# lppllppl920/SAGE-SLAM

Measured on AMD Instinct MI355X. Metric: M residuals/sec (+ LM iters/sec), 64-keyframe feature-metric BA @128x160, higher is better.
Workload: dtype f32; 1 GPU; 64-keyframe window, 128x160x16 feature pyramids (L=4), 32-dim depth code, dense sampling N=16128, 186 links = 372 photometric + 372 geometric directed edges; parallelism=single GPU, collective=none, accepted_steps=988

## Files before the change

include/sage_ba.h:

```cpp
#ifndef SAGE_BA_H_
#define SAGE_BA_H_

#include <stddef.h>
#include <stdint.h>

#ifdef __cplusplus
extern "C" {
#endif

#define SAGE_MAX_LEVELS 8
#define SAGE_POSE_FLOATS 12

#define SAGE_OK 0
#define SAGE_E_INVALID (-1)
#define SAGE_E_UNSUPPORTED (-2)
#define SAGE_E_NOT_PSD (-3)
#define SAGE_E_STATE (-4)
#define SAGE_E_NO_OVERLAP (-5)

typedef struct SageCamera
{
  float fx, fy, cx, cy, w, h;
} SageCamera;

// ... 621 lines not shown
                                        const float *matched_2d, const SageCamera *cam, float eps, float loss_param,
                                        float weight, int N);

enum { SAGE_LOSS_FAIR = 0, SAGE_LOSS_L2 = 1, SAGE_LOSS_HUBER = 2, SAGE_LOSS_UNBIASED = 3 };
int sage_match_geometry_jac_error_calculate(SageWorkspace *ws, float *AtA_dev, float *Atb_dev, float *error_host,
                                            const float *R10, const float *t10, const float *R0, const float *t0,
                                            const float *R1, const float *t1, const float *bias0, const float *bias1,
                                            const float *basis0, const float *basis1, const float *code0,
                                            const float *code1, const float *homo0, const float *matched_homo1,
                                            const int32_t *loc1d_0, const int32_t *matched_loc1d_1, float scale0,
                                            float scale1, float loss_param, float weight, int loss, int N, int CS);
int sage_match_geometry_error_calculate(SageWorkspace *ws, float *error_host, const float *R10, const float *t10,
                                        const float *bias0, const float *bias1, const float *basis0, const float *basis1,
                                        const float *code0, const float *code1, const float *homo0,
                                        const float *matched_homo1, const int32_t *loc1d_0,
                                        const int32_t *matched_loc1d_1, float scale0, float scale1, float loss_param,
                                        float weight, int loss, int N, int CS);
int sage_loop_mg_jac_error_calculate(SageWorkspace *ws, float *AtA_dev, float *Atb_dev, float *error_host,
                                     const float *R10, const float *t10, const float *R0, const float *t0,
                                     const float *R1, const float *t1, const float *unscaled_dpts0,
                                     const float *matched_unscaled_dpts1, const float *homo0, const float *matched_homo1,
                                     float scale0, float scale1, float loss_param, float weight, int N);
int sage_loop_mg_error_calculate(SageWorkspace *ws, float *error_host, const float *R10, const float *t10,
                                 const float *unscaled_dpts0, const float *matched_unscaled_dpts1, const float *homo0,
                                 const float *matched_homo1, float scale0, float scale1, float loss_param, float weight,
                                 int N);
int sage_tracker_match_geom_jac_error_calculate(SageWorkspace *ws, float *AtA_dev, float *Atb_dev, float *error_host,
                                                const float *R, const float *t, const float *sampled_dpts0,
                                                const float *matched_dpts1, const float *homo0,
                                                const float *matched_homo1, float scale0, float loss_param,
                                                float weight, int with_scale, int N);
int sage_tracker_match_geom_error_calculate(SageWorkspace *ws, float *error_host, const float *R, const float *t,
                                            const float *sampled_dpts0, const float *matched_dpts1, const float *homo0,
                                            const float *matched_homo1, float loss_param, float weight, int N);

int sage_cycle_match(SageWorkspace *ws, const float *desc0_dev, const float *desc1_dev, const int64_t *kp_loc1d_0,
                     int K, int C, int H, int W, float cyc_thresh, int64_t *raw_matched_loc1d_1,
                     int64_t *cyc_matched_loc1d_0, int32_t *inlier_flags, int *n_inliers_host);

int sage_sort_locations(SageWorkspace *ws, const int64_t *loc1d_dev, const float *homo_dev, int n, int H, int W,
                        int64_t *loc1d_out_dev, float *homo_out_dev, int *sorted_host);
int sage_valid_locations(SageWorkspace *ws, const float *mask_dev, const SageCamera *cam, int64_t *loc1d_dev,
                         float *homo_dev, int *n_valid_host);
int sage_shuffle_indices(int64_t seed, int64_t n, int64_t *idx_host);
int sage_sample_locations(SageWorkspace *ws, const int64_t *valid_loc1d_dev, const float *valid_homo_dev, int n_valid,
                          int64_t seed, int num_samples, int64_t *loc1d_dev, float *homo_dev, int *n_out_host);

typedef int (*SageAllReduceFn)(double *dev_buf, size_t n, void *user);
int sage_window_set_allreduce(SageWindow *w, SageAllReduceFn fn, void *user);

typedef struct SageShardPlan SageShardPlan;
int sage_shard_plan_create(int K, int nlinks, const int32_t *links, int B, int rank, int world, SageShardPlan **out);
void sage_shard_plan_destroy(SageShardPlan *p);
size_t sage_shard_sep_count(const SageShardPlan *p);
int sage_shard_num_separators(const SageShardPlan *p);
int sage_shard_num_interior(const SageShardPlan *p);
int sage_shard_keyframe_owner(const SageShardPlan *p, int kf);
int sage_shard_keyframe_is_local(const SageShardPlan *p, int kf);
int sage_shard_eliminate(SageShardPlan *p, const double *packed_local_host, double damp, const double *diag_add,
                         const double *g_add, double *sep_out);
int sage_shard_solve(SageShardPlan *p, const double *sep_reduced, double *delta);
int sage_shard_plan_create_domains(int K, int nlinks, const int32_t *links, int B, int domain, int ndomains,
                                   SageShardPlan **out);
int sage_block_solve_domains(const double *packed_host, int K, int nlinks, const int32_t *links, int B, double damp,
                             const double *diag_add, const double *g_add, int ndomains, double *delta);

int sage_window_emulate_peers(SageWindow *w, const double *rest_dev, int n_iterates);
#define SAGE_RCCL_ID_BYTES 128
int sage_rccl_unique_id(unsigned char *id128);
int sage_rccl_comm_create(const unsigned char *id128, int rank, int world, void **comm_out);
void sage_rccl_comm_destroy(void *comm);
int sage_rccl_comm_info(void *comm, int *ranks_out, int *rank_out);
int sage_window_use_rccl(SageWindow *w, void *nccl_comm);

typedef struct SageLmState
{
  double damp, error, candidate_error;
  int accepted, iters;
} SageLmState;
int sage_window_lm_step(SageWindow *w, SageLmState *st, const SageLmConfig *cfg);
int sage_window_lm_run(SageWindow *w, SageLmState *st, const SageLmConfig *cfg, int n, double *trace, int *done);
int sage_window_lm_run_timed(SageWindow *w, SageLmState *st, const SageLmConfig *cfg, int n, double *trace, int *done,
                             double *step_seconds);
int sage_window_sync_variables(SageWindow *w);

enum { SAGE_DOGLEG_SEARCH_EACH_ITERATION = 0, SAGE_DOGLEG_SEARCH_REDUCE_ONLY = 1, SAGE_DOGLEG_ONE_STEP_PER_ITERATION = 2 };
typedef struct SageDoglegConfig
{
  double init_delta;
  double min_delta;
  int mode;
} SageDoglegConfig;
void sage_dogleg_config_default(SageDoglegConfig *cfg);
typedef struct SageDoglegState
{
  double delta, error, candidate_error, rho, step_norm, sd_norm, gn_norm, a, b;
  double dots[6];
  int region, accepted, evals, solves, iters;
} SageDoglegState;
int sage_dogleg_point(double delta, double gg, double gn, double nn, double gAg, double *a, double *b, int *region);
typedef int (*SageDoglegEvalFn)(void *ctx, double a, double b, double *f_candidate);
int sage_dogleg_iterate(const SageDoglegConfig *cfg, const double *dots, double f_error, SageDoglegEvalFn eval, void *ctx,
                        SageDoglegState *st);
int sage_dogleg_incidence(int K, int nlinks, const int32_t *links, int32_t *offsets, int32_t *entries);

int sage_window_dogleg_step(SageWindow *w, SageDoglegState *st, const SageDoglegConfig *cfg);
int sage_window_dogleg_run(SageWindow *w, SageDoglegState *st, const SageDoglegConfig *cfg, int n, double *trace, int *done);
int sage_window_dogleg_products(SageWindow *w, double *dots);
int sage_window_dogleg_candidate(SageWindow *w, double a, double b);
int sage_window_get_dogleg_vectors(SageWindow *w, double *g, double *Ag, double *n, double *An);

#ifdef __cplusplus
}
#endif
#endif
```

sage_slam_amd/build.py:

```python
from __future__ import annotations

import os
import subprocess
import sys
from concurrent.futures import ThreadPoolExecutor

HERE = os.path.dirname(os.path.abspath(__file__))
ROOT = os.path.dirname(HERE)
CSRC = os.path.join(HERE, "csrc")
OBJ = os.path.join(HERE, "csrc", "_obj")
LIB = os.path.join(HERE, "libsage_ba.so")
SOURCES = ["photo_kernels.hip", "geo_kernels.hip", "track_kernels.hip", "producers.hip", "keypoint_kernels.hip", "graph_kernels.hip", "solve_kernels.hip", "operators.hip", "tracker.hip", "overlap.hip", "depth_scale.hip", "bow.hip", "registration.hip", "match_batch.hip", "voc_build.hip", "window.hip", "window_eval.hip", "window_reduce.hip", "window_solve.hip", "window_lm.hip", "window_profile.hip", "window_build.hip", "window_terms.hip", "window_dist.hip", "window_factors.hip", "psd_project.hip", "window_dogleg.hip",
           "host_math.cpp", "factor_blocks.cpp", "block_solver.cpp", "host_threads.cpp", "shard_solve.cpp", "convex_hull.cpp", "bow_database.cpp", "registration_host.cpp", "voc_build_host.cpp", "depth_scale_host.cpp", "loop_accept_host.cpp", "psd_project_host.cpp", "dogleg_host.cpp"]
HEADERS = ["sage_device.h", "sage_internal.h", "damped_system.h", "host_math.h", "factor_blocks.h", "block_solver.h", "host_threads.h", "device_buffers.h", "runtime_internal.h", "window_state.h", "finalize_bodies.h", "keypoint_batch.h", "graph_terms.h", "graph_batch.h", "term_results.h", "window_plan.h", "registration_plan.h", "registration_math.h", "depth_scale_plan.h", "loop_accept.h", "voc_build.h", "psd_project.h", "dogleg.h", os.path.join(ROOT, "include", "sage_ba.h")]
HIPCC = os.environ.get("HIPCC", "/opt/rocm/bin/hipcc")
HOSTCXX = os.environ.get("HOSTCXX", "/opt/rocm/lib/llvm/bin/clang++")
FLAGS = ["--offload-arch=gfx950", "-O3", "-std=c++17", "-fPIC", "-Wall", "-Wno-unused-function",
         "-I" + os.path.join(ROOT, "include"), "-I" + CSRC]


def kernel_source_sha16() -> str:
    import hashlib
    h = hashlib.sha256()
    for f in ("photo_kernels.hip", "geo_kernels.hip", "sage_device.h", "sage_internal.h"):
        with open(os.path.join(CSRC, f), "rb") as fh:
            h.update(fh.read())
    return h.hexdigest()[:16]


def _mtime(p):
    return os.path.getmtime(p) if os.path.exists(p) else 0.0


def _compile(src):
    obj = os.path.join(OBJ, os.path.splitext(src)[0] + ".o")
    deps = [os.path.join(CSRC, src)] + [h if os.path.isabs(h) else os.path.join(CSRC, h) for h in HEADERS]
    if _mtime(obj) >= max(_mtime(d) for d in deps):
        return obj, False
    if src.endswith(".hip"):
        cmd = [HIPCC] + FLAGS + ["-x", "hip", "-c", os.path.join(CSRC, src), "-o", obj]
    else:
        cmd = [HOSTCXX, "-O3", "-std=c++17", "-fPIC", "-Wall", "-I" + os.path.join(ROOT, "include"), "-I" + CSRC,
               "-c", os.path.join(CSRC, src), "-o", obj]
    subprocess.check_call(cmd)
    return obj, True


def build(force: bool = False, verbose: bool = False) -> str:
    os.makedirs(OBJ, exist_ok=True)
    if force:
        for f in os.listdir(OBJ):
            os.remove(os.path.join(OBJ, f))
    with ThreadPoolExecutor(max_workers=min(8, len(SOURCES))) as ex:
        res = list(ex.map(_compile, SOURCES))
    objs = [o for o, _ in res]
    if any(ch for _, ch in res) or not os.path.exists(LIB):
        subprocess.check_call([HIPCC, "--offload-arch=gfx950", "-shared", "-fPIC", "-o", LIB] + objs + ["-lpthread"])
        if verbose:
            print("built", LIB)
    return LIB


GLUE_SRC = os.path.join(ROOT, "integration", "compile_check", "prepass_run.cpp")
GLUE_BIN = os.path.join(ROOT, "integration", "compile_check", "_bin", "prepass_run")
REF_THIRDPARTY = "/root/reference/system/thirdparty"


def build_glue_check(verbose: bool = False):
    if not os.path.isdir(REF_THIRDPARTY):
        return GLUE_BIN if os.path.exists(GLUE_BIN) else None
    deps = [GLUE_SRC, os.path.join(ROOT, "integration", "sage_gtsam_prepass.h"), os.path.join(ROOT, "include", "sage_ba.h"),
            os.path.join(ROOT, "integration", "compile_check", "gtsam", "linear", "HessianFactor.h"),
            os.path.join(ROOT, "integration", "compile_check", "gtsam", "nonlinear", "Values.h"), LIB]
    if _mtime(GLUE_BIN) >= max(_mtime(d) for d in deps):
        return GLUE_BIN
    os.makedirs(os.path.dirname(GLUE_BIN), exist_ok=True)
    subprocess.check_call([HOSTCXX, "-std=c++17", "-O1", "-w", "-D__HIP_PLATFORM_AMD__", "-I" + os.path.join(ROOT, "include"),
                           "-I" + os.path.join(ROOT, "integration", "compile_check"), "-I" + REF_THIRDPARTY + "/eigen",
                           "-I" + REF_THIRDPARTY + "/Sophus", "-I/opt/rocm/include", GLUE_SRC, "-o", GLUE_BIN,
                           "-L" + HERE, "-lsage_ba", "-L/opt/rocm/lib", "-lamdhip64",
                           "-Wl,-rpath,$ORIGIN/../../../sage_slam_amd", "-Wl,-rpath,/opt/rocm/lib"])
    if verbose:
        print("built", GLUE_BIN)
    return GLUE_BIN


ADAPTER_BIN = os.path.join(ROOT, "integration", "compile_check", "_bin", "adapter_run")
REF_SYSTEM = "/root/reference/system"


def build_adapter_run(verbose: bool = False):
    if not os.path.isdir(REF_SYSTEM):
        return ADAPTER_BIN if os.path.exists(ADAPTER_BIN) else None
    import torch
    T = os.path.dirname(torch.__file__)
    srcs = [os.path.join(ROOT, "integration", "sage_adapter.cpp"), os.path.join(ROOT, "integration", "sage_adapter_keypoints.cpp"),
            os.path.join(ROOT, "integration", "compile_check", "adapter_run.cpp")]
# ... 31 lines not shown
```

sage_slam_amd/capi.py:

```python
from __future__ import annotations

import ctypes as C
import os
from typing import List, Optional, Sequence

import numpy as np

HERE = os.path.dirname(os.path.abspath(__file__))
LIB_PATH = os.path.join(HERE, "libsage_ba.so")
SAGE_MAX_LEVELS = 8


class SageError(RuntimeError):
    def __init__(self, code: int, where: str):
        self.code = code
        msg = lib().sage_error_string(code).decode() if _lib is not None else "?"
        super().__init__(f"{where}: {msg} (code {code})")


class SageCamera(C.Structure):
    _fields_ = [(n, C.c_float) for n in ("fx", "fy", "cx", "cy", "w", "h")]


class SagePyramid(C.Structure):
# ... 87 lines not shown


SAGE_DOGLEG_SEARCH_EACH_ITERATION, SAGE_DOGLEG_SEARCH_REDUCE_ONLY, SAGE_DOGLEG_ONE_STEP_PER_ITERATION = 0, 1, 2
DOGLEG_DOTS = ("gg", "gn", "nn", "gAg", "gAn", "nAn")


class SageDoglegConfig(C.Structure):
    _fields_ = [("init_delta", C.c_double), ("min_delta", C.c_double), ("mode", C.c_int)]


class SageDoglegState(C.Structure):
    _fields_ = [(n, C.c_double) for n in ("delta", "error", "candidate_error", "rho", "step_norm", "sd_norm", "gn_norm", "a", "b")] + \
               [("dots", C.c_double * 6)] + \
               [(n, C.c_int) for n in ("region", "accepted", "evals", "solves", "iters")]


DOGLEG_EVAL_FN = C.CFUNCTYPE(C.c_int, C.c_void_p, C.c_double, C.c_double, C.POINTER(C.c_double))


def dogleg_config_default() -> SageDoglegConfig:
    cfg = SageDoglegConfig()
    lib().sage_dogleg_config_default(C.byref(cfg))
    return cfg


def dogleg_point(delta, gg, gn, nn, gAg):
    f = lib().sage_dogleg_point
    f.argtypes = [C.c_double] * 5 + [C.c_void_p] * 3
    a, b, region = C.c_double(), C.c_double(), C.c_int()
    rc = int(f(delta, gg, gn, nn, gAg, C.addressof(a), C.addressof(b), C.addressof(region)))
    return rc, a.value, b.value, region.value


def dogleg_iterate(cfg: SageDoglegConfig, dots, f_error, fn, state: SageDoglegState) -> int:
    d = np.ascontiguousarray(dots, np.float64)
    assert d.size == 6

    def tramp(_ctx, a, b, out):
        try:
            out[0] = float(fn(a, b))
            return 0
        except Exception:
            import traceback
            traceback.print_exc()
            return -4

    f = lib().sage_dogleg_iterate
    f.argtypes = [C.c_void_p, C.c_void_p, C.c_double, DOGLEG_EVAL_FN, C.c_void_p, C.c_void_p]
    return int(f(C.addressof(cfg), d.ctypes.data, float(f_error), DOGLEG_EVAL_FN(tramp), None, C.addressof(state)))


def dogleg_incidence(K: int, links):
    lk = np.ascontiguousarray(np.asarray(links, np.int32).reshape(-1, 2))
    off = np.zeros(max(K, 0) + 1, np.int32)
    ent = np.zeros((max(K, 0) + 2 * len(lk), 2), np.int32)
    f = lib().sage_dogleg_incidence
    f.argtypes = [C.c_int, C.c_int, C.c_void_p, C.c_void_p, C.c_void_p]
    rc = int(f(int(K), len(lk), lk.ctypes.data if len(lk) else None, off.ctypes.data, ent.ctypes.data))
    return rc, off, ent


TRACK_LIN_FN = C.CFUNCTYPE(C.c_int, C.c_void_p, C.POINTER(C.c_float), C.c_float, C.POINTER(C.c_float),
                           C.POINTER(C.c_float), C.POINTER(C.c_float))
TRACK_ERR_FN = C.CFUNCTYPE(C.c_int, C.c_void_p, C.POINTER(C.c_float), C.c_float, C.POINTER(C.c_float))

_lib = None

SYMBOLS = [
    "sage_camera_pyramid", "sage_version", "sage_error_string", "sage_workspace_create", "sage_workspace_destroy",
    "sage_photometric_jac_error_calculate", "sage_photometric_error_calculate",
    "sage_tracker_photo_jac_error_calculate", "sage_tracker_photo_error_calculate",
    "sage_geometric_jac_error_calculate", "sage_geometric_error_calculate", "sage_depth_and_grad",
    "sage_gaussian_pyramid_with_grad", "sage_se3_exp", "sage_pose_retract", "sage_nearest_psd", "sage_nearest_psd_reference", "sage_factor_block_count", "sage_factor_hessian_blocks",
    "sage_damped_solve_qr_f32", "sage_block_solve", "sage_solve_lookahead_count", "sage_lm_config_default", "sage_track_lm", "sage_track_lm_batch", "sage_track_frame", "sage_track_frame_batch", "sage_track_overlap", "sage_track_overlap_batch", "sage_track_overlap_batch_plan", "sage_track_overlap_batch_launches", "sage_convex_hull_area", "sage_depth_scale_ratio", "sage_median_f32",
    "sage_depth_scale_ratio_batch", "sage_median_f32_batch", "sage_depth_scale_ratio_batch_plan", "sage_depth_scale_ratio_batch_launches",
    "sage_vocabulary_create", "sage_vocabulary_destroy", "sage_vocabulary_num_nodes", "sage_vocabulary_num_words", "sage_vocabulary_channels", "sage_vocabulary_depth", "sage_vocabulary_max_fanout", "sage_vocabulary_staged_nodes",
    "sage_vocabulary_build_config_default", "sage_vocabulary_build", "sage_vocabulary_build_desc", "sage_vocabulary_build_docs_with_word", "sage_vocabulary_build_node_of_point", "sage_vocabulary_build_stats", "sage_vocabulary_build_plan", "sage_vocabulary_build_draw", "sage_vocabulary_build_destroy",
    "sage_bow_transform", "sage_bow_score", "sage_bow_db_create", "sage_bow_db_destroy", "sage_bow_db_add", "sage_bow_db_size", "sage_bow_db_query",
    "sage_window_create", "sage_window_destroy", "sage_window_add_keyframe", "sage_window_add_link", "sage_window_add_keypoint_link", "sage_window_hold", "sage_window_set_link_geo_loss",
    "sage_window_set_shard", "sage_window_finalize", "sage_window_num_keyframes", "sage_window_num_links",
    "sage_window_block_size", "sage_window_solver_block_size", "sage_window_packed_count", "sage_window_packed_dev",
    "sage_window_residuals_per_linearize", "sage_window_bytes_per_linearize", "sage_window_linearize",
    "sage_window_error", "sage_window_tune_runs", "sage_window_set_runs", "sage_window_error_dev", "sage_window_solve", "sage_window_total_error",
    "sage_window_accept", "sage_window_reset", "sage_window_get_keyframe", "sage_window_set_keyframe", "sage_window_get_delta",
    "sage_window_get_edge", "sage_window_add_keypoint_term", "sage_window_num_keypoint_terms", "sage_window_get_keypoint_term", "sage_window_add_graph_term", "sage_window_num_graph_terms", "sage_window_get_graph_term", "sage_window_prepass", "sage_window_factor", "sage_window_factor_error", "sage_term_factor_block_count", "sage_term_factor_blocks", "sage_window_keypoint_factor", "sage_window_keypoint_factor_error", "sage_window_graph_factor", "sage_window_graph_factor_error", "sage_window_prepare_factors", "sage_window_prepare_factors_device", "sage_window_prepare_factors_device_launches", "sage_factor_psd", "sage_factor_psd_batch", "sage_factor_psd_batch_launches", "sage_factor_psd_batch_plan", "sage_jacobi_round_pairs", "sage_factor_cut_blocks", "sage_window_set_profiling", "sage_window_get_kernel_time", "sage_window_get_phase_time", "sage_window_lm_step", "sage_window_lm_run", "sage_window_lm_run_timed", "sage_window_sync_variables", "sage_window_set_allreduce", "sage_shard_plan_create", "sage_shard_plan_create_domains", "sage_block_solve_domains", "sage_shard_plan_destroy", "sage_shard_sep_count", "sage_shard_num_separators", "sage_shard_num_interior", "sage_shard_keyframe_owner", "sage_shard_keyframe_is_local", "sage_shard_eliminate", "sage_shard_solve", "sage_rccl_unique_id", "sage_rccl_comm_create", "sage_rccl_comm_destroy", "sage_rccl_comm_info", "sage_window_use_rccl", "sage_window_emulate_peers", "sage_sort_locations", "sage_bind_thread_to_device", "sage_solver_helper_cpus", "sage_solver_placement_moves", "sage_placement_monitor", "sage_shutdown", "sage_host_threads_running",
    "sage_valid_locations", "sage_shuffle_indices", "sage_sample_locations",
    "sage_reprojection_jac_error_calculate", "sage_reprojection_error_calculate",
    "sage_tracker_reproj_jac_error_calculate", "sage_tracker_reproj_error_calculate",
    "sage_match_geometry_jac_error_calculate", "sage_match_geometry_error_calculate",
    "sage_loop_mg_jac_error_calculate", "sage_loop_mg_error_calculate",
    "sage_tracker_match_geom_jac_error_calculate", "sage_tracker_match_geom_error_calculate", "sage_cycle_match",
    "sage_robust_registration", "sage_tls_estimate", "sage_registration_finish", "sage_match_points",
    "sage_cycle_match_batch", "sage_cycle_match_batch_slices", "sage_loop_precheck", "sage_loop_verify", "sage_loop_accept",
    "sage_robust_registration_batch", "sage_robust_registration_batch_plan", "sage_robust_registration_batch_launches",
    "sage_match_points_batch",
    "sage_workspace_set_registration_finish", "sage_workspace_registration_finish", "sage_registration_finish_batch",
    "sage_registration_finish_plan",
    "sage_dogleg_config_default", "sage_dogleg_point", "sage_dogleg_iterate", "sage_dogleg_incidence",
    "sage_window_dogleg_step", "sage_window_dogleg_run", "sage_window_dogleg_products", "sage_window_dogleg_candidate",
    "sage_window_get_dogleg_vectors",
]


def lib():
    global _lib
    if _lib is None:
        LIB_PATH = os.environ.get("SAGE_BA_LIB", globals()["LIB_PATH"])
        if not os.path.exists(LIB_PATH):
            raise ImportError(f"{LIB_PATH} is missing: run `python -m sage_slam_amd.build` "
                              "(the HIP engine has no fallback path)")
        import torch
        L = C.CDLL(LIB_PATH)
        L.sage_version.restype = C.c_char_p
        L.sage_error_string.restype = C.c_char_p
        L.sage_window_packed_count.restype = C.c_size_t
        L.sage_shutdown.restype = None
        L.sage_window_packed_dev.restype = C.c_void_p
        L.sage_window_error_dev.restype = C.c_void_p
        L.sage_window_residuals_per_linearize.restype = C.c_double
        L.sage_window_bytes_per_linearize.restype = C.c_double
        for name in ("sage_window_packed_count", "sage_window_packed_dev", "sage_window_error_dev",
                     "sage_window_residuals_per_linearize", "sage_window_bytes_per_linearize",
                     "sage_window_num_keyframes", "sage_window_num_links", "sage_window_block_size",
                     "sage_window_solver_block_size"):
            getattr(L, name).argtypes = [C.c_void_p]
        _lib = L
    return _lib


def _chk(code: int, where: str):
    if code != 0:
        raise SageError(code, where)


def _f32(a) -> np.ndarray:
    return np.ascontiguousarray(a, dtype=np.float32)


def _fp(a: np.ndarray):
    return a.ctypes.data_as(C.POINTER(C.c_float))


def dptr(t) -> C.c_void_p:
    if t is None:
        return C.c_void_p(0)
    assert t.is_contiguous(), "device buffers handed to the C ABI must be contiguous"
    return C.c_void_p(t.data_ptr())


def make_pyramid(cam, levels: int) -> SagePyramid:
    base = SageCamera(*[float(v) for v in (cam.fx, cam.fy, cam.cx, cam.cy, cam.w, cam.h)])
    out = SagePyramid()
    _chk(lib().sage_camera_pyramid(C.byref(base), levels, C.byref(out)), "sage_camera_pyramid")
    return out


def se3_exp(omega, v):
    omega = _f32(omega); v = _f32(v)
    R = np.zeros(9, np.float32); t = np.zeros(3, np.float32)
    lib().sage_se3_exp(_fp(omega), _fp(v), _fp(R), _fp(t))
    return R.reshape(3, 3), t


def pose_retract(pose12, delta6):
    pose12 = _f32(pose12).reshape(12); delta6 = _f32(delta6)
    out = np.zeros(12, np.float32)
    lib().sage_pose_retract(_fp(pose12), _fp(delta6), _fp(out))
# ... 1089 lines not shown
    def tune_runs(self):
        tpb, rule = C.c_int(0), C.c_int(0)
        ms_rule, ms_best = C.c_float(0), C.c_float(0)
        _chk(lib().sage_window_tune_runs(self.h, C.byref(tpb), C.byref(rule), C.byref(ms_rule), C.byref(ms_best)),
             "sage_window_tune_runs")
        return dict(tpb=tpb.value, tpb_rule=rule.value, ms_rule=ms_rule.value, ms_best=ms_best.value)

    def set_runs(self, tpb):
        _chk(lib().sage_window_set_runs(self.h, int(tpb)), "sage_window_set_runs")

    def solve(self, damp, want_norm=True):
        if not want_norm:
            _chk(lib().sage_window_solve(self.h, C.c_double(damp), None), "sage_window_solve")
            return None
        sn = C.c_double()
        _chk(lib().sage_window_solve(self.h, C.c_double(damp), C.byref(sn)), "sage_window_solve")
        return sn.value

    def total_error(self, from_linearize: bool):
        e = C.c_double()
        _chk(lib().sage_window_total_error(self.h, int(from_linearize), C.byref(e)), "sage_window_total_error")
        return e.value

    def accept(self):
        _chk(lib().sage_window_accept(self.h), "sage_window_accept")

    def reset(self):
        _chk(lib().sage_window_reset(self.h), "sage_window_reset")

    def set_allreduce(self, dist_module, group=None):
        tensors = {}
        for t in (self.packed_tensor(), self.error_tensor()):
            tensors[(t.data_ptr(), t.numel())] = t

        def hook(ptr, n, _user):
            try:
                t = tensors.get((ptr, n))
                if t is None:
                    t = tensors[(ptr, n)] = _tensor_from_ptr(ptr, n)
                dist_module.all_reduce(t, group=group)
                return 0
            except Exception:
                import traceback
                traceback.print_exc()
                return 1

        self._allreduce_cb = ALLREDUCE_FN(hook)
        _chk(lib().sage_window_set_allreduce(self.h, self._allreduce_cb, None), "sage_window_set_allreduce")

    def sync_variables(self):
        _chk(lib().sage_window_sync_variables(self.h), "sage_window_sync_variables")

    def use_rccl(self, comm):
        _chk(lib().sage_window_use_rccl(self.h, C.c_void_p(comm)), "sage_window_use_rccl")

    def emulate_peers(self, rest):
        if rest is None:
            self._emu_rest = None
            _chk(lib().sage_window_emulate_peers(self.h, None, 0), "sage_window_emulate_peers")
            return
        assert rest.is_cuda and rest.dim() == 2 and rest.shape[1] == self.packed_count and rest.is_contiguous()
        self._emu_rest = rest
        _chk(lib().sage_window_emulate_peers(self.h, C.c_void_p(rest.data_ptr()), int(rest.shape[0])),
             "sage_window_emulate_peers")

    def lm_step(self, state: SageLmState, cfg: SageLmConfig):
        _chk(lib().sage_window_lm_step(self.h, C.byref(state), C.byref(cfg)), "sage_window_lm_step")
        return state

    def lm_run(self, state: SageLmState, cfg: SageLmConfig, n: int):
        tr = np.zeros((n, 4), np.float64)
        done = C.c_int()
        _chk(lib().sage_window_lm_run(self.h, C.byref(state), C.byref(cfg), n, tr.ctypes.data_as(C.POINTER(C.c_double)),
                                      C.byref(done)), "sage_window_lm_run")
        return tr[:done.value]

    def lm_run_timed(self, state: SageLmState, cfg: SageLmConfig, n: int):
        tr = np.zeros((n, 4), np.float64); sec = np.zeros(n, np.float64)
        done = C.c_int()
        _chk(lib().sage_window_lm_run_timed(self.h, C.byref(state), C.byref(cfg), n, tr.ctypes.data_as(C.POINTER(C.c_double)),
                                            C.byref(done), sec.ctypes.data_as(C.POINTER(C.c_double))), "sage_window_lm_run_timed")
        return tr[:done.value], sec[:done.value]

    def dogleg_step(self, state: SageDoglegState, cfg: SageDoglegConfig):
        _chk(lib().sage_window_dogleg_step(self.h, C.byref(state), C.byref(cfg)), "sage_window_dogleg_step")
        return state

    def dogleg_run(self, state: SageDoglegState, cfg: SageDoglegConfig, n: int):
        tr = np.zeros((n, 7), np.float64)
        done = C.c_int()
        _chk(lib().sage_window_dogleg_run(self.h, C.byref(state), C.byref(cfg), n, tr.ctypes.data_as(C.POINTER(C.c_double)),
                                          C.byref(done)), "sage_window_dogleg_run")
        return tr[:done.value]

    def dogleg_products(self):
        d = np.zeros(6, np.float64)
        _chk(lib().sage_window_dogleg_products(self.h, d.ctypes.data_as(C.POINTER(C.c_double))), "sage_window_dogleg_products")
        return d

    def dogleg_candidate(self, a, b):
        f = lib().sage_window_dogleg_candidate
        f.argtypes = [C.c_void_p, C.c_double, C.c_double]
        _chk(f(self.h, float(a), float(b)), "sage_window_dogleg_candidate")

    def dogleg_vectors(self):
        v = [np.zeros(self.K * self.B, np.float64) for _ in range(4)]
        _chk(lib().sage_window_get_dogleg_vectors(self.h, *[x.ctypes.data_as(C.POINTER(C.c_double)) for x in v]),
             "sage_window_get_dogleg_vectors")
        return tuple(v)

    def delta(self):
        d = np.zeros(self.K * self.B, np.float64)
        _chk(lib().sage_window_get_delta(self.h, d.ctypes.data_as(C.POINTER(C.c_double))), "sage_window_get_delta")
        return d

    def get_keyframe(self, k):
        pose = np.zeros(12, np.float32); code = np.zeros(self.win.CS, np.float32); s = C.c_float()
        _chk(lib().sage_window_get_keyframe(self.h, k, _fp(pose), _fp(code), C.byref(s)), "sage_window_get_keyframe")
        return pose, code, s.value

    def set_keyframe(self, k, pose12, code, scale):
        pose12 = _f32(pose12); code = _f32(code)
        _chk(lib().sage_window_set_keyframe(self.h, k, _fp(pose12), _fp(code), C.c_float(scale)),
             "sage_window_set_keyframe")

    def get_edge(self, type_, e):
        D = 13 + self.win.CS if type_ == 0 else 14 + 2 * self.win.CS
        A = np.zeros((D, D), np.float32); b = np.zeros(D, np.float32)
        err = C.c_float(); nin = C.c_float()
        _chk(lib().sage_window_get_edge(self.h, type_, e, _fp(A), _fp(b), C.byref(err), C.byref(nin)),
             "sage_window_get_edge")
        return dict(AtA=A, Atb=b, error=err.value, num_inliers=nin.value)

    def prepass(self, poses12, codes, scales, jacobians: bool = True) -> bool:
        P = _f32(np.asarray(poses12).reshape(-1)); Cd = _f32(np.asarray(codes).reshape(-1)); S = _f32(np.asarray(scales).reshape(-1))
        K = self.K
        assert P.size == K * 12 and Cd.size == K * self.win.CS and S.size == K
        rec = C.c_int32()
        _chk(lib().sage_window_prepass(self.h, _fp(P), _fp(Cd), _fp(S), int(jacobians), C.byref(rec)), "sage_window_prepass")
        return bool(rec.value)

    _FACTOR_ARGTYPES = {n: [C.c_void_p] + [C.c_int] * (n + 1) + [C.c_void_p] * 5 for n in (1, 2)}
    _ERROR_ARGTYPES = {n: [C.c_void_p] + [C.c_int] * n + [C.c_void_p] for n in (1, 2)}

    def _cached_factor(self, name, ids, psd_mode, check):
        f_ = getattr(lib(), name)
        f_.argtypes = self._FACTOR_ARGTYPES[len(ids)]
        D = 14 + 2 * self.win.CS
        G = np.zeros(D * (D + 1) // 2 + D * D, np.float64); g = np.zeros(D, np.float64); f = C.c_double()
        dims = (C.c_int32 * 6)(); nk = C.c_int32()
        rc = int(f_(self.h, *ids, int(psd_mode), G.ctypes.data, g.ctypes.data, C.addressof(f), C.addressof(dims), C.addressof(nk)))
        if rc != 0:
            if check:
                raise SageError(rc, name)
            return rc, None
        dims = [int(dims[k]) for k in range(nk.value)]
        blocks, gs = _blocks_of(G, g[:sum(dims)].copy(), dims)
        out = (blocks, gs, f.value, dims)
        return out if check else (rc, out)

    def _cached_error(self, name, ids, check):
        f_ = getattr(lib(), name)
        f_.argtypes = self._ERROR_ARGTYPES[len(ids)]
        v = C.c_double()
        rc = int(f_(self.h, *ids, C.addressof(v)))
        if check:
# ... 877 lines not shown
```

sage_slam_amd/csrc/block_solver.cpp:

```cpp
#include <algorithm>
#include <atomic>
#include <chrono>
#include <cmath>
#include <cstdio>
#include <cstdlib>
#include <cstring>
#include <sched.h>
#include <thread>
#include <vector>

#include "block_solver.h"
#include "damped_system.h"
#include "host_math.h"
#include "sage_ba.h"

namespace sage
{
namespace
{
typedef double v8d __attribute__((vector_size(64), aligned(8)));

#define SAGE_LOADU(dst, p) __builtin_memcpy(&(dst), (p), sizeof(v8d))
#define SAGE_STOREU(p, v) __builtin_memcpy((p), &(v), sizeof(v8d))

// ... 219 lines not shown
template <int NV, int CB>
static inline __attribute__((always_inline)) void inverse_rows(const double *S, double *X, const double *rinv)
{
  constexpr int BP = NV * 8;
  for (int cc = 7; cc >= 0; --cc)
  {
    const int c = 8 * CB + cc;
    double e[8] = {0, 0, 0, 0, 0, 0, 0, 0};
    e[cc] = 1.0;
    v8d a0[NV], a1[NV];
#pragma unroll
    for (int v = 0; v < NV; ++v)
      a0[v] = a1[v] = v8d{0, 0, 0, 0, 0, 0, 0, 0};
    SAGE_LOADU(a0[CB], e);
    const double *u = S + c * BP;
    for (int t = c + 1; t < 8 * CB + 8; ++t)
    {
      const double f = u[t];
      const v8d fv = {f, f, f, f, f, f, f, f};
#pragma unroll
      for (int v = CB; v < NV; ++v)
      {
        v8d x;
        SAGE_LOADU(x, X + t * BP + 8 * v);
        a0[v] -= fv * x;
      }
    }
    if constexpr (CB + 1 < NV)
      inverse_accumulate<NV, CB + 1>(u, X, a0, a1);
    const double inv = rinv[c];
    const v8d iv = {inv, inv, inv, inv, inv, inv, inv, inv};
#pragma unroll
    for (int v = 0; v < NV; ++v)
    {
      v8d r = (a0[v] + a1[v]) * iv;
      SAGE_STOREU(X + c * BP + 8 * v, r);
    }
  }
  if constexpr (CB > 0)
    inverse_rows<NV, CB - 1>(S, X, rinv);
}

template <int NV>
static inline __attribute__((always_inline)) bool factor_diag(double *S, double *X)
{
  constexpr int BP = NV * 8;
  double rinv[BP];
  if (!factor_panel<NV, 0>(S, rinv))
    return false;
  inverse_rows<NV, NV - 1>(S, X, rinv);
  return true;
}

template <int NV>
struct Blocks
{
  const BlockEnvelope &E;
  double *T;
  inline __attribute__((always_inline)) double *operator()(int i, int j) const { return T + E.index(i, j) * (size_t)(NV * 8 * NV * 8); }
};

template <int NV>
static inline __attribute__((always_inline)) RowPrefetch row_prefetch(const BlockEnvelope &E, const double *T, int r)
{
  constexpr size_t BB = (size_t)NV * 8 * NV * 8;
  const BlockEnvelope::Range a = E.a_range(r);
  const size_t b0 = (size_t)(a.hi > a.lo ? E.a_off[r] : E.row_off[r]);
  const size_t nb = (size_t)(a.hi - a.lo) + (size_t)(r - E.row_first[r] + 1);
  const char *p = reinterpret_cast<const char *>(T + b0 * BB);
  return RowPrefetch{p, p + nb * BB * sizeof(double)};
}

static inline __attribute__((always_inline)) bool wait_block(const BlockEnvelope &E, double *T, size_t idx,
                                                             std::atomic<int> *abort = nullptr, bool peek = false)
{
  const size_t BB = (size_t)E.Bp * E.Bp;
  if (E.fill && E.fill[idx])
  {
    std::memset(T + idx * BB, 0, BB * sizeof(double));
    return true;
  }
  if (!E.ready)
    return true;
  const volatile unsigned *f = E.ready + idx;
  if (!peek || *f != E.epoch)
  {
    const double t0 = mono_seconds();
    unsigned spins = 0;
    while (*f != E.epoch)
    {
      __builtin_ia32_pause();
      if ((++spins & 0xfff) == 0 && ((abort && abort->load(std::memory_order_acquire)) || mono_seconds() - t0 > 2.0))
      {
        if (abort)
          abort->store(2, std::memory_order_release);
        return false;
      }
    }
  }
  std::atomic_thread_fence(std::memory_order_acquire);
  return true;
}

static __attribute__((noinline)) bool wait_row_tickets(const BlockEnvelope &E, int i, double *T, int from_col = 0,
                                                       int skip_lo = 0, int skip_hi = 0)
{
  const BlockEnvelope::Range rg[2] = {E.a_range(i), {E.row_first[i], i + 1}};
  for (int r = 0; r < 2; ++r)
    for (int j = rg[r].lo; j < rg[r].hi; ++j)
      if (j >= from_col && !(j >= skip_lo && j < skip_hi) && !wait_block(E, T, E.index(i, j), nullptr, true))
        return false;
  return true;
}

#define SAGE_HSUM8(a) ((((a)[0] + (a)[4]) + ((a)[1] + (a)[5])) + (((a)[2] + (a)[6]) + ((a)[3] + (a)[7])))

template <int NV>
static inline __attribute__((always_inline)) void fwd_sub_block(double *w, const double *Tk, const double *yk)
{
  constexpr int BP = NV * 8;
  for (int t = 0; t < BP; ++t)
  {
    const double f = yk[t];
    for (int r = 0; r < BP; ++r)
      w[r] -= f * Tk[t * BP + r];
  }
}

template <int NV>
static inline __attribute__((always_inline)) void apply_diag_inverse(double *y_i, const double *w, const double *Xi)
{
  constexpr int BP = NV * 8;
  double yi[BP];
  for (int c = 0; c < BP; ++c)
    yi[c] = 0.0;
  for (int t = 0; t < BP; ++t)
  {
    const double f = w[t];
    for (int c = 0; c < BP; ++c)
      yi[c] += f * Xi[t * BP + c];
  }
  for (int c = 0; c < BP; ++c)
    y_i[c] = yi[c];
}

template <int NV>
static inline __attribute__((always_inline)) void backsub_columns(double *z, Blocks<NV> blk, const double *y, int i,
                                                                  const int32_t *rows, int nrows, int skip_from)
{
  constexpr int BP = NV * 8;
  for (int t0 = 0; t0 < BP; t0 += 8)
  {
    v8d acc[8];
    for (int u = 0; u < 8; ++u)
      acc[u] = v8d{0, 0, 0, 0, 0, 0, 0, 0};
    for (int q = 0; q < nrows; ++q)
    {
      const int m = rows ? rows[q] : i + 1 + q;
      if (m >= skip_from)
        break;
      if (!rows && !blk.E.has(m, i))
        continue;
      const double *Tm = blk(m, i) + t0 * BP, *xm = y + (size_t)m * BP;
      for (int v = 0; v < NV; ++v)
      {
        v8d xv;
        SAGE_LOADU(xv, xm + 8 * v);
        for (int u = 0; u < 8; ++u)
        {
          v8d a;
          SAGE_LOADU(a, Tm + u * BP + 8 * v);
          acc[u] += a * xv;
// ... 848 lines not shown
            job.ta.size(), job.tb.size(), 1e6 * (mono_seconds() - t_halves));
  if (rc == 0 && job.abort.load(std::memory_order_acquire))
    rc = -2;
  return rc ? rc : sep_finish_bp(job.E->Bp, job);
}

static void arrow_back_substitute(SepJob &job, BlockEnvelope &E, int rc)
{
  const bool par_c = rc == 0 && !job.tc.empty();
  job.goC.store(par_c ? 1 : 2, std::memory_order_release);
  if (!par_c)
    return;
  sep_work_c(job, false);
  while (job.doneC.load(std::memory_order_acquire) < (int)job.tc.size())
    cpu_relax();
  E.bs_skip_from = job.sep0;
}

void CholHelper::run(int)
{
  int expect = 0;
  if (!claim.compare_exchange_strong(expect, 1, std::memory_order_acq_rel))
    return;
  const BlockEnvelope &e = *E;
  if (kind == 1)
  {
    const int rc = block_chol_range(e, T, X, y, lo, hi, RowRole::lookahead);
    p1_rc.store(rc == -2 ? -3 : rc, std::memory_order_release);
    return;
  }
  const bool piped = lookahead_engage(2, e, T, X, y, e.n1, e.n1 + e.n2);
  const int rc = block_chol_range(e, T, X, y, e.n1, e.n1 + e.n2, piped ? RowRole::chain : RowRole::whole);
  if (piped)
    lookahead_release(2);
  p1_rc.store(rc, std::memory_order_release);
  int g;
  while ((g = go_p2.load(std::memory_order_acquire)) == 0)
    cpu_relax();
  if (g == 1)
    block_back_range(e, T, X, y, e.n1, e.n1 + e.n2);
  p2_done.store(1, std::memory_order_release);
}
}

Worker *solve_worker(int idx, bool make)
{
  if (idx < 3)
    return chol_helper(idx);
  return make ? sep_pool() : g_sep_pool_made.load(std::memory_order_acquire);
}


int block_plan_long_arrow_chains(const BlockEnvelope &E)
{
  int n = 0;
  if (E.n1 > 0 && E.n2 > 0 && E.a_cnt)
    for (int i = E.n1 + E.n2; i < E.K; ++i)
      for (int h = 0; h < 2; ++h)
        n += E.sep_range(i, h).hi - E.sep_range(i, h).lo > 16 ? 1 : 0;
  return n;
}

bool block_plan_has_arrow_rows(const BlockEnvelope &E)
{
  long long reach = 0;
  if (E.n1 > 0 && E.n2 > 0 && E.a_cnt)
    for (int i = E.n1 + E.n2; i < E.K; ++i)
      for (int h = 0; h < 2; ++h)
        reach += E.sep_range(i, h).hi - E.sep_range(i, h).lo;
  return reach > 64;
}

int plan_blocks(int K, const std::vector<std::pair<int, int>> &links, bool may_split, BlockPlan &out)
{
  std::vector<int32_t> &perm = out.perm, &pos = out.pos, &row_first = out.row_first, &row_off = out.row_off,
                       &a_first = out.a_first, &a_cnt = out.a_cnt, &a_off = out.a_off, &blk_row = out.blk_row,
                       &blk_col = out.blk_col, &blk_src = out.blk_src;
  int &n1 = out.n1, &n2 = out.n2, &nblk = out.nblk;
  perm.assign(K, 0);
  pos.assign(K, 0);
  for (int k = 0; k < K; ++k)
    perm[k] = k;
  n1 = n2 = 0;
  for (auto &l : links)
    if (l.first < 0 || l.second <= l.first || l.second >= K)
      return SAGE_E_INVALID;
  if (may_split && K >= 16)
  {
    constexpr int bias = 1;
    std::vector<char> inC(K, 0);
    std::vector<int> cover;
    int best_m = -1, best_w = 0;
    for (;;)
    {
      int best_cost = 2 * K;
      best_m = -1;
      for (int m = K / 4; m <= (3 * K) / 4; ++m)
      {
        int wdt = 0;
        for (auto &l : links)
          if (!inC[l.first] && !inC[l.second] && l.first < m && l.second >= m)
            wdt = std::max(wdt, l.second - m + 1);
        if (wdt < 1 || wdt > 8 || m + wdt > K - 2)
          continue;
        const int cost = std::max(m, K - m - wdt + bias) + 2 * wdt;
        if (cost < best_cost)
        {
          best_cost = cost;
          best_m = m;
          best_w = wdt;
        }
      }
      if (best_m > 0 || cover.size() >= 8)
        break;
      std::vector<int> deg(K, 0);
      int any = 0;
      for (auto &l : links)
        if (!inC[l.first] && !inC[l.second] && l.second - l.first > 8)
        {
          ++deg[l.first];
          ++deg[l.second];
          ++any;
        }
      if (!any)
        break;
      const int pick = (int)(std::max_element(deg.begin(), deg.end()) - deg.begin());
      inC[pick] = 1;
      cover.push_back(pick);
    }
    if (best_m > 0)
    {
      int q = 0;
      for (int k = 0; k < best_m; ++k)
        if (!inC[k])
          perm[q++] = k;
      n1 = q;
      for (int k = K - 1; k >= best_m + best_w; --k)
        if (!inC[k])
          perm[q++] = k;
      n2 = q - n1;
      for (int k = best_m; k < best_m + best_w; ++k)
        if (!inC[k])
          perm[q++] = k;
      std::sort(cover.begin(), cover.end());
      for (int k : cover)
        perm[q++] = k;
      if (n1 < 1 || n2 < 1)
      {
        for (int k = 0; k < K; ++k)
          perm[k] = k;
        n1 = n2 = 0;
      }
    }
  }
  for (int q = 0; q < K; ++q)
    pos[perm[q]] = q;
  const bool split = n1 > 0;
  const int sep0 = n1 + n2;
  row_first.assign(K, 0);
  row_off.assign(K, 0);
  a_first.assign(K, 0);
  a_cnt.assign(K, 0);
  a_off.assign(K, 0);
  for (int k = 0; k < K; ++k)
  {
    row_first[k] = k;
    a_first[k] = n1;
  }
  for (auto &l : links)
  {
    const int i = std::max(pos[l.first], pos[l.second]), j = std::min(pos[l.first], pos[l.second]);
    if (split && i >= sep0 && j < n1)
      a_first[i] = std::min(a_first[i], j);
    else
      row_first[i] = std::min(row_first[i], j);
  }
  if (split)
    for (int i = sep0; i < K; ++i)
    {
      row_first[i] = std::min(row_first[i], (int32_t)sep0);
      a_cnt[i] = n1 - a_first[i];
    }
  nblk = 0;
  for (int k = 0; k < K; ++k)
  {
    a_off[k] = nblk;
    nblk += a_cnt[k];
    row_off[k] = nblk;
    nblk += k - row_first[k] + 1;
  }
  blk_row.assign(nblk, 0);
  blk_col.assign(nblk, 0);
  blk_src.assign(nblk, -1);
  for (int k = 0; k < K; ++k)
  {
    for (int j = a_first[k]; j < a_first[k] + a_cnt[k]; ++j)
    {
      blk_row[out.index(k, j)] = k;
      blk_col[out.index(k, j)] = j;
    }
    for (int j = row_first[k]; j <= k; ++j)
    {
      blk_row[out.index(k, j)] = k;
      blk_col[out.index(k, j)] = j;
    }
  }
  out.col_ptr.assign(K + 1, 0);
  for (int b = 0; b < nblk; ++b)
    if (blk_row[b] != blk_col[b])
      ++out.col_ptr[blk_col[b] + 1];
  for (int j = 0; j < K; ++j)
    out.col_ptr[j + 1] += out.col_ptr[j];
  out.col_rows.assign(std::max(1, (int)out.col_ptr[K]), 0);
  {
    std::vector<int32_t> fill(out.col_ptr.begin(), out.col_ptr.end() - 1);
    for (int k = 0; k < K; ++k)
    {
      for (int j = a_first[k]; j < a_first[k] + a_cnt[k]; ++j)
        out.col_rows[fill[j]++] = k;
      for (int j = row_first[k]; j < k; ++j)
        out.col_rows[fill[j]++] = k;
    }
  }
  for (size_t l = 0; l < links.size(); ++l)
  {
    const int a = links[l].first, b = links[l].second;
    const int i = std::max(pos[a], pos[b]), j = std::min(pos[a], pos[b]);
    int &src = blk_src[out.index(i, j)];
    if (src >= 0)
      return SAGE_E_UNSUPPORTED;
    src = (int)l | (perm[i] == a ? 0x40000000 : 0);
  }
  return SAGE_OK;
}
// ... 181 lines not shown
```

sage_slam_amd/csrc/block_solver.h:

```cpp
#pragma once
#include <stdint.h>

#include <algorithm>
#include <atomic>
#include <utility>
#include <vector>

#include "host_threads.h"

namespace sage
{
inline int padded_block(int B) { return B < 1 ? 0 : B <= 8 ? 8 : B <= 24 ? 24 : B <= 40 ? 40 : 0; }

struct BlockEnvelope
{
  int K = 0, Bp = 0;
  const int32_t *row_first = nullptr, *row_off = nullptr;
  const int32_t *a_first = nullptr, *a_cnt = nullptr, *a_off = nullptr;
  int n1 = 0, n2 = 0;
  const volatile unsigned *ready = nullptr;
  unsigned epoch = 0;
  const uint8_t *fill = nullptr;
  bool no_lookahead = false;
  std::atomic<int> *progress = nullptr;
  const int32_t *col_ptr = nullptr, *col_rows = nullptr;
  int bs_skip_from = 0x7fffffff;
  struct RowPipe
  {
    alignas(64) std::atomic<int> early{0};
    alignas(64) std::atomic<int> late{0};
    alignas(64) std::atomic<int> pre{0};
  };
  RowPipe *pipe = nullptr;
  bool sep_pre = false;

  struct Range
  {
    int lo, hi;
  };
  Range a_range(int i) const
  {
    const int a = a_cnt ? a_first[i] : 0;
    return {a, a + (a_cnt ? a_cnt[i] : 0)};
  }
  Range b_range(int i) const { return {row_first[i], i}; }
  bool has(int i, int j) const
  {
    const Range a = a_range(i);
    return (j >= row_first[i] && j <= i) || (j >= a.lo && j < a.hi);
  }
  size_t index(int i, int j) const
  {
    return (size_t)(j < row_first[i] ? a_off[i] + j - a_first[i] : row_off[i] + j - row_first[i]);
  }
  double *block(double *T, int i, int j) const { return T + index(i, j) * (size_t)(Bp * Bp); }
  Range sep_range(int srow, int half) const
  {
    if (half == 0)
      return a_range(srow);
    const int sep0 = n1 + n2;
    return {std::min((int)row_first[srow], sep0), sep0};
  }
};
int block_chol_solve_tr(const BlockEnvelope &env, double *T, double *X, double *y);
int block_chol_partial(const BlockEnvelope &env, double *T, double *X, double *y, int nI);
int block_chol_partial_back(const BlockEnvelope &env, double *T, double *X, double *y, int nI);
int block_plan_long_arrow_chains(const BlockEnvelope &env);
bool block_plan_has_arrow_rows(const BlockEnvelope &env);

struct BlockPlan
{
  std::vector<int32_t> perm, pos, row_first, row_off, a_first, a_cnt, a_off, blk_row, blk_col, blk_src;
  std::vector<int32_t> col_ptr, col_rows;
  int nblk = 0, n1 = 0, n2 = 0;
  int index(int i, int j) const
  {
    return j < row_first[i] ? a_off[i] + j - a_first[i] : row_off[i] + j - row_first[i];
  }
};
int plan_blocks(int K, const std::vector<std::pair<int, int>> &links, bool may_split, BlockPlan &out);
BlockEnvelope envelope_of(const BlockPlan &plan, int Bp);
}
```

sage_slam_amd/csrc/runtime_internal.h:

```cpp
#pragma once

#include <hip/hip_runtime.h>

#include <algorithm>
#include <atomic>
#include <cctype>
#include <sched.h>
#include <chrono>
#include <cmath>
#include <cstddef>
#include <cstdlib>
#include <cstdio>
#include <cstring>
#include <thread>
#include <vector>

#include <dlfcn.h>
#if __has_include(<rccl/rccl.h>)
#include <rccl/rccl.h>
#else
extern "C"
{
  typedef struct ncclComm *ncclComm_t;
  typedef struct
  {
    char internal[128];
  } ncclUniqueId;
  typedef enum { ncclSuccess = 0 } ncclResult_t;
  typedef enum { ncclSum = 0 } ncclRedOp_t;
  typedef enum { ncclDouble = 8 } ncclDataType_t;
}
#endif

#include "device_buffers.h"
#include "host_math.h"
#include "factor_blocks.h"
#include "host_threads.h"
#include "sage_ba.h"
#include "sage_internal.h"
#include "keypoint_batch.h"
#include "graph_batch.h"
#include "window_plan.h"
#include "registration_plan.h"
#include "depth_scale_plan.h"
#include "loop_accept.h"
#include "dogleg.h"

using namespace sage;

#define SAGE_HIP(expr)                \
  do                                  \
  {                                   \
    hipError_t _e = (expr);           \
    if (_e != hipSuccess)             \
      return (int)_e;                 \
  } while (0)

namespace sage_rt
{

inline int pick_tiles_per_block(long long total_tiles)
{
  if (total_tiles >= 8192)
    return 4;
  if (total_tiles >= 4096)
    return 2;
  return 1;
}

struct WorkList
{
  std::vector<WorkItem> work;
  std::vector<int32_t> edge_first, edge_tiles;
  std::vector<int32_t> rec_first, rec_count;
  int tiles_per_block = 1;
  int flush = 1;
  int n_records = 0;
  void build(const std::vector<int> &N, int tpb_override = 0, const std::vector<int> *order = nullptr, int flush_ = 0)
  {
    long long total = 0;
    for (int n : N)
      total += (n + kTile - 1) / kTile;
    tiles_per_block = tpb_override > 0 ? tpb_override : pick_tiles_per_block(total);
    flush = (flush_ > 0 && flush_ < tiles_per_block && tiles_per_block % flush_ == 0) ? flush_ : tiles_per_block;
    work.clear();
    edge_first.assign(N.size(), 0);
    edge_tiles.assign(N.size(), 0);
    rec_first.assign(N.size(), 0);
    rec_count.assign(N.size(), 0);
    n_records = 0;
    for (size_t i = 0; i < N.size(); ++i)
    {
      const size_t e = order ? (size_t)(*order)[i] : i;
      const int tiles = (N[e] + kTile - 1) / kTile;
      edge_first[e] = (int32_t)work.size();
      for (int t = 0; t < tiles; t += tiles_per_block)
        work.push_back(WorkItem{(int32_t)e, t});
      edge_tiles[e] = (int32_t)work.size() - edge_first[e];
      rec_first[e] = n_records;
      rec_count[e] = (tiles + flush - 1) / flush;
      n_records += rec_count[e];
    }
  }
};

template <class Pred>
inline bool spin_until(Pred done)
{
  const auto t0 = std::chrono::steady_clock::now();
  unsigned spins = 0;
  while (!done())
  {
    __builtin_ia32_pause();
    if ((++spins & 0x3ff) == 0 && std::chrono::duration<double>(std::chrono::steady_clock::now() - t0).count() > 0.05)
      return false;
  }
  std::atomic_thread_fence(std::memory_order_acquire);
  return true;
}

}
using namespace sage_rt;

struct WsHostStats
{
  float stats[4];
  float pad[4];
  unsigned ticket;
  unsigned tail[7];
// ... 38 lines not shown
  bool sel_scratch_zero = false;
  int sel_batch_launches = 0;
  DevBuf bow_hit;
  PinnedBuf bow_host;
  bool bow_hit_zero = false;
  DevBuf reg_keys, reg_payload, reg_pairs, reg_tiles;
  PinnedBuf reg_host;
  int reg_batch_launches = 0;
  int reg_finish_mode = 0;
  DevBuf mb_part, mb_done;
  PinnedBuf mb_host;
  int mb_cus = 0, mb_slices = 0;
  DevBuf pre_scratch;
  PinnedBuf psd_host;
  int psd_launches = 0;

  WsHostStats *hs() const { return host_stats.as<WsHostStats>(); }
  TrackHost *trk() const { return trk_host.as<TrackHost>(); }
};

int ws_ticket_wait(SageWorkspace *ws);
unsigned ws_ticket_next(SageWorkspace *ws);
int ws_ticket_await(SageWorkspace *ws, unsigned epoch);
int track_photo_enqueue(SageWorkspace *ws, bool jac, int dof, float *AtA, float *Atb, float *stats, const float *R,
                        const float *t, const float *mask1, const float *dpts0, const float *homo, const float *feat0s,
                        const float *feat1, const float *grad1, const SagePyramid *pyr, float scale0, float eps,
                        const float *weights_dev, int N, int FS);
int track_reproj_enqueue(SageWorkspace *ws, bool jac, float *AtA, float *Atb, float *stats, const float *R, const float *t,
                         const float *sampled_dpts0, const float *homo, const float *matched_2d, const SageCamera *cam,
                         float eps, float loss_param, float weight, int N);
int track_match_geom_enqueue(SageWorkspace *ws, int mode, bool jac, float *AtA, float *Atb, float *stats, const float *R,
                             const float *t, const float *sampled_dpts0, const float *matched_dpts1, const float *homo0,
                             const float *matched_homo1, float scale0, float loss_param, float weight, int N);

int psd_project_enqueue(hipStream_t s, int D, int n, const float *AtA_dev, double *C_dev, SagePsdStats *stats);

int registration_check_params(const SageRegistrationParams *p);

static inline bool supported(int CS, int FS)
{
  return (CS == 16 || CS == 32) && (FS == 16 || FS == 32);
}

namespace sage
{
struct AdjEntry
{
  int32_t type;
  int32_t edge;
  int32_t role;
};

struct LinkEdges
{
  int32_t e_ab, e_ba;
};

struct AssembleParams
{
  const float *AtA_p, *Atb_p, *stats_p;
  const float *AtA_g, *Atb_g, *stats_g;
  const double *wide_p, *wide_g;
  const int32_t *adj_start;
  const AdjEntry *adj;
  const LinkEdges *links;
  double *packed;
  double *tail_mirror;
  int K, nlinks, CS, n_edges_p, n_edges_g;
  int split;
  const int32_t *blocks;
  const int32_t *link_terms_start;
  const AdjEntry *link_terms;
  TermResults terms;
};

struct ErrorTotalsSide
{
  const int32_t *edge_first, *edge_tiles;
  const float *partials;
  float *stats;
  float fallback, scale;
  int n_edges;
  int stride, err_off, cnt_off;
};

}

#include "window_state.h"

struct SageWindow
{
  SageWindowConfig cfg;
  hipStream_t stream = nullptr;
  bool finalized = false;
  int rank = 0, world = 1;
  int K = 0, B = 0, VS = 0;
  std::vector<SageKeyframeView> views;
  HostVars hv;
  std::vector<float> link_geo_loss;
  std::vector<std::pair<int, int>> links;
  std::vector<char> link_dense;
  std::vector<uint8_t> hold;
  sage::plan::SolverRows rows;
  std::vector<int> local_links;
  std::vector<int> owned_edges;
  std::vector<int> local_edges;
  int n_edges = 0;
  DevBuf vars[2];
  DevBuf sorted_loc, sorted_homo;
  std::vector<std::pair<const int64_t *, const float *>> user_samples;
  std::vector<int> user_n;
  DevBuf dpt, dgrad, depth_items[2];
  int n_depth = 0;
  int dpt_set = -1;
  bool dgrad_valid = false;
  DevBuf geo_px;
  bool merge_ok = false;
  DevBuf pk;
  DevBuf f0s;
  DenseSide dense[2];
  PhotoRecordPlan photo_rec;
  std::vector<int> Nedge;
  int tpb_heur = 1;
  DevBuf adj_start, adj, link_edges, packed, errbuf;
  TotalsMirror mirror;
  WindowDist dist;
  std::vector<double> host_packed;
  std::vector<double> delta;
  sage::DeviceSolver *solver = nullptr;
  bool cand_pending = false;
  double residuals_per_lin = 0, bytes_per_lin = 0;
  bool have_lin = false;
  uint64_t vars_epoch = 1, lin_epoch = 0;
  bool spec_err_valid = false;
  double spec_error = 0.0;
  DevBuf packed_save;
  TermSide terms;
  FactorCache fc;
  uint64_t dense_serial = 0;
  DoglegSide dogleg;
  WindowProfiler prof;

  bool kernels_mirror_totals() const { return world == 1 && !dist.allreduce && mirror.h; }
};


template <class T>
static int upload(DevBuf &b, const std::vector<T> &v, hipStream_t s)
{
  int rc = b.reserve(std::max<size_t>(v.size(), 1) * sizeof(T));
  if (rc)
    return rc;
  if (!v.empty())
    SAGE_HIP(hipMemcpyAsync(b.p, v.data(), v.size() * sizeof(T), hipMemcpyHostToDevice, s));
  return 0;
}
int window_upload_vars(SageWindow *w, int set);
int window_local_edge(const SageWindow *w, int global_edge);
bool window_owns_edge(const SageWindow *w, int global_edge);
bool window_has_holds(const SageWindow *w);
std::vector<int32_t> window_link_pairs(const SageWindow *w);
struct FinalizeState
{
  bool domain_solve = false;
  std::vector<char> needed;
  std::vector<size_t> f0s_off;
  std::vector<size_t> px_off;
  std::vector<int> Nedge;
  std::vector<std::vector<AdjEntry>> adjv;
  std::vector<LinkEdges> le;
  std::vector<char> link_terms;
  double residuals = 0, bytes = 0;
};
int finalize_terms(SageWindow *w, FinalizeState &fs);
int window_launch_terms(SageWindow *w, int set, bool jac);
int window_linearize_set(SageWindow *w, int set, double *dst = nullptr, bool local_blocks = false, bool merge = false);
int window_error_pass(SageWindow *w, int which, bool speculate_gradients);
int window_collective(SageWindow *w, double *buf, size_t n);
int window_allreduce(SageWindow *w, double *buf, size_t n, int iterate);
int window_allreduce_into(SageWindow *w, const double *send, double *recv, size_t n, int iterate);
int window_mirror_totals(SageWindow *w, bool with_err, const double *system = nullptr);
bool window_wait_error_totals(SageWindow *w);
bool window_wait_reduced_totals(SageWindow *w);
int window_wait_mirror(SageWindow *w, bool *not_psd);
double mirrored_error(const SageWindow *w, int at, int set);
int window_total_error(SageWindow *w, int from_linearize, double *err, bool stream_idle);
int window_copy_floats(SageWindow *w, const float *src, float *dst, int n);
void window_add_to_double(SageWindow *w, double *p, double v);
double window_prior_error(const SageWindow *w, int set, bool owned_only = false);
SolvePriors window_solve_priors(const SageWindow *w);
int window_sync_candidate(SageWindow *w, bool stream_idle = false);
int window_schur_solve(SageWindow *w, double damp, double *lin_error);
void prof_attach(SageWindow *w, int which, LaunchCommon &lc);
void window_phase_mark(SageWindow *w, int which);
```

sage_slam_amd/csrc/solve_kernels.hip:

```cpp
#include <algorithm>
#include <atomic>
#include <chrono>
#include <cstdio>
#include <cstring>
#include <memory>
#include <vector>

#include "block_solver.h"
#include "device_buffers.h"
#include "damped_system.h"
#include "host_math.h"
#include "sage_device.h"
#include "sage_internal.h"
#include "window_plan.h"

namespace sage
{

struct SolvePlan
{
  int K, B, Bs, Bp, nblk, nlinks;
  const int32_t *row_first;
  const int32_t *row_off;
  const int32_t *blk_row, *blk_col, *blk_src;
  const int32_t *perm, *pos;
  const int32_t *hold;
  const int32_t *to_block, *to_solver;
};

struct SolveResult
{
  double step_norm2;
  int status;
  unsigned go;
};
static size_t result_vars_offset() { return sizeof(SolveResult); }
static size_t result_delta_offset(int K, int VS) { return (sizeof(SolveResult) + (size_t)K * VS * sizeof(float) + 15) / 16 * 16; }

constexpr int kScatterWorkgroups = 32;

__global__ __launch_bounds__(256) void solve_scatter_kernel(const SolvePlan P, const double *__restrict__ packed,
                                                            const float *__restrict__ vars0, int VS, int CS,
                                                            const SolvePriors pri, double damp,
                                                            double *__restrict__ L, double *__restrict__ y,
                                                            const int32_t *__restrict__ order, unsigned *flags,
                                                            unsigned epoch)
{
  const int tid = threadIdx.x;
  const int B = P.B, Bs = P.Bs, Bp = P.Bp, BB = B * B;
  __shared__ double s_dadd[64], s_gadd[64];
  __shared__ int s_row[64];
  if (tid < Bs)
    s_row[tid] = P.to_block[tid];
  __syncthreads();
  for (int it = blockIdx.x; it < P.nblk; it += gridDim.x)
  {
    const int b = order[it];
    const int i = P.blk_row[b], j = P.blk_col[b], srcf = P.blk_src[b];
    const int src = srcf < 0 ? -1 : (srcf & 0x3fffffff);
    const bool row_is_a = srcf >= 0 && (srcf & 0x40000000);
    if (src < 0 && i != j)
      continue;
    const int kf = P.perm[i];
    const int hold_r = P.hold ? P.hold[kf] : 0, hold_c = P.hold ? P.hold[P.perm[j]] : 0;
    const double *diag = packed + (size_t)kf * BB;
    const double *lnk = packed + (size_t)P.K * BB + (size_t)(src < 0 ? 0 : src) * BB;
    const double *g = packed + (size_t)P.K * BB + (size_t)P.nlinks * BB + (size_t)kf * B;
    double *out = L + (size_t)b * Bp * Bp;
    if (i == j)
    {
      const float *var = vars0 + (size_t)kf * VS;
      if (tid < Bs)
      {
        double da, ga;
        prior_row(pri, kf, s_row[tid], CS, var, var[12], var + 13, da, ga, hold_r);
        s_dadd[tid] = da;
        s_gadd[tid] = ga;
      }
      __syncthreads();
    }
    for (int o = tid; o < Bp * Bp; o += blockDim.x)
    {
      const int c = o / Bp, r = o - c * Bp;
      double v = 0.0;
      const bool in = r < Bs && c < Bs;
      const bool held = in && solver_elem_held(hold_r, hold_c, s_row, r, c, CS);
      if (i == j)
        v = in ? (held ? held_diag_elem(r, c) : solver_diag_elem(diag, B, s_row, r, c, s_dadd[r], damp))
               : damped_pad_elem(r, c, damp);
      else if (in && !held)
        v = lnk[solver_link_elem(row_is_a, s_row, r, c, B)];
      out[o] = v;
    }
    if (i == j)
      for (int r = tid; r < Bp; r += blockDim.x)
        y[(size_t)i * Bp + r] =
            (r < Bs && !(hold_r && row_held(hold_r, s_row[r], CS))) ? damped_rhs_elem(g[s_row[r]], s_gadd[r]) : 0.0;
    __syncthreads();
    if (tid == 0)
    {
      __threadfence_system();
      *reinterpret_cast<volatile unsigned *>(flags + b) = epoch;
    }
  }
}

__global__ __launch_bounds__(1024) void solve_retract_kernel(const double *__restrict__ x, int K, int B, int Bp, int CS,
                                                            int VS, const int32_t *__restrict__ pos,
                                                            const int32_t *__restrict__ hold,
                                                            const int32_t *__restrict__ to_solver,
                                                            const float *__restrict__ vars0,
                                                            float *__restrict__ vars1, float *__restrict__ h_vars,
                                                            double *__restrict__ h_delta, SolveResult *h_res,
                                                            unsigned epoch)
{
  const int tid = threadIdx.x;
  const volatile unsigned *go = &h_res->go;
  __shared__ int s_go;
  if (tid == 0)
  {
    const unsigned long long t0 = wall_clock64();
    unsigned v;
    bool timed_out = false;
    for (;;)
    {
      v = *go;
      const unsigned d = ((v & 0x7fffffffu) - epoch) & 0x7fffffffu;
      if (d == 0u)
        break;
      if (d < 0x40000000u && (v & 0x7fffffffu) != 0u)
      {
        v = 0x80000000u;
        break;
      }
      __builtin_amdgcn_s_sleep(4);
      if (wall_clock64() - t0 > 200000000ull)
      {
        v = 0x80000000u;
// ... 13 lines not shown
  for (int idx = tid; idx < K * B; idx += blockDim.x)
  {
    const int k = idx / B, r = idx - k * B;
    const bool held = hold && row_held(hold[k], r, CS);
    const double d = held ? 0.0 : x[(size_t)pos[k] * Bp + to_solver[r]];
    h_delta[idx] = d;
    nrm += d * d;
    const float *v0 = vars0 + (size_t)k * VS;
    if (r >= 6)
    {
      const int slot = r < 6 + CS ? 13 + r - 6 : 12;
      const float v = held ? v0[slot] : v0[slot] + (float)d;
      vars1[(size_t)k * VS + slot] = v;
      h_vars[(size_t)k * VS + slot] = v;
    }
  }
  for (int k = tid; k < K; k += blockDim.x)
  {
    const double *xk = x + (size_t)pos[k] * Bp;
    const float *v0 = vars0 + (size_t)k * VS;
    float *o = vars1 + (size_t)k * VS;
    if (hold && (hold[k] & kHoldPose))
      for (int i = 0; i < 12; ++i)
        o[i] = v0[i];
    else
    {
      float d6[6];
      for (int i = 0; i < 6; ++i)
        d6[i] = (float)xk[to_solver[i]];
      pose_retract(v0, d6, o);
    }
    for (int i = 0; i < 12; ++i)
      h_vars[(size_t)k * VS + i] = o[i];
  }
  __shared__ double s_n[16];
  for (int off = 32; off > 0; off >>= 1)
    nrm += __shfl_down(nrm, off);
  if ((tid & 63) == 0)
    s_n[tid >> 6] = nrm;
  __syncthreads();
  if (tid == 0)
  {
    double tot = 0.0;
    for (int w = 0; w < (int)(blockDim.x >> 6); ++w)
      tot += s_n[w];
    h_res->step_norm2 = tot;
  }
}

struct DeviceSolver
{
  int K = 0, B = 0, Bs = 0, Bp = 0, nblk = 0, nlinks = 0, VS = 0;
  sage_rt::DevBuf d_int;
  sage_rt::DevBuf d_hold;
  sage_rt::PinnedBuf h_pinned;
  sage_rt::PinnedBuf h_T;
  double *h_y = nullptr;
  unsigned *h_flags = nullptr;
  unsigned epoch = 0, go_epoch = 0;
  SolvePlan plan{};
  const int32_t *d_order = nullptr;
  std::vector<double> h_X;
  BlockPlan host_plan;
  std::vector<uint8_t> h_fill;

  double *h_blocks() const { return h_T.as<double>(); }
  SolveResult *result() const { return h_pinned.as<SolveResult>(); }
  float *host_vars() const { return reinterpret_cast<float *>(h_pinned.as<char>() + result_vars_offset()); }
  double *host_delta() const { return reinterpret_cast<double *>(h_pinned.as<char>() + result_delta_offset(K, VS)); }
};

int solver_create(DeviceSolver **out, int K, const plan::SolverRows &rows, int VS,
                  const std::vector<std::pair<int, int>> &links, hipStream_t stream)
{
  *out = nullptr;
  const int B = rows.B, Bs = rows.Bs;
  const int Bp = sage::padded_block(Bs);
  if (Bp == 0 || K < 1)
    return SAGE_E_UNSUPPORTED;
  BlockPlan bp;
  const int rcp = plan_blocks(K, links, !sage::env_flag("SAGE_SOLVE_NO_SPLIT"), bp);
  if (rcp != SAGE_OK)
    return rcp;
  const int n1 = bp.n1, n2 = bp.n2, nblk = bp.nblk;
  const std::vector<int32_t> &perm = bp.perm, &pos = bp.pos, &row_first = bp.row_first, &row_off = bp.row_off,
                             &a_cnt = bp.a_cnt, &a_off = bp.a_off, &blk_row = bp.blk_row, &blk_col = bp.blk_col,
                             &blk_src = bp.blk_src;
  std::unique_ptr<DeviceSolver> S(new DeviceSolver);
  S->K = K; S->B = B; S->Bs = Bs; S->Bp = Bp; S->nblk = nblk; S->nlinks = (int)links.size(); S->VS = VS;
  std::vector<int32_t> all;
  auto put = [&](const std::vector<int32_t> &v) {
    const size_t off = all.size();
    all.insert(all.end(), v.begin(), v.end());
    while (all.size() % 4)
      all.push_back(0);
    return off;
  };
  const size_t o_rf = put(row_first), o_ro = put(row_off), o_br = put(blk_row), o_bc = put(blk_col),
               o_bs = put(blk_src), o_pm = put(perm), o_ps = put(pos);
  std::vector<int32_t> order;
  auto push_row = [&](int i) {
    for (int q = 0; q < a_cnt[i]; ++q)
      order.push_back(a_off[i] + q);
    for (int q = 0; q <= i - row_first[i]; ++q)
      order.push_back(row_off[i] + q);
  };
  if (n1 > 0)
  {
    for (int t = 0; t < std::max(n1, n2); ++t)
    {
      if (t < n1)
        push_row(t);
      if (t < n2)
        push_row(n1 + t);
    }
    for (int i = n1 + n2; i < K; ++i)
      push_row(i);
  }
  else
    for (int i = 0; i < K; ++i)
      push_row(i);
  const size_t o_ord = put(order);
  const size_t o_tb = put(rows.to_block), o_ts = put(rows.to_solver);
  if (S->d_int.reserve(all.size() * sizeof(int32_t)))
    return (int)hipErrorOutOfMemory;
  if (hipMemcpyAsync(S->d_int.p, all.data(), all.size() * sizeof(int32_t), hipMemcpyHostToDevice, stream) != hipSuccess)
    return (int)hipErrorUnknown;
  if (hipStreamSynchronize(stream) != hipSuccess)
    return (int)hipErrorUnknown;
  const size_t ty_doubles = (size_t)nblk * Bp * Bp + (size_t)K * Bp;
  if (S->h_T.reserve(ty_doubles * sizeof(double) + (size_t)nblk * sizeof(unsigned)))
    return (int)hipErrorOutOfMemory;
  S->h_y = S->h_blocks() + (size_t)nblk * Bp * Bp;
  S->h_flags = reinterpret_cast<unsigned *>(S->h_blocks() + ty_doubles);
  std::memset(S->h_flags, 0, (size_t)nblk * sizeof(unsigned));
  S->h_X.assign((size_t)K * Bp * Bp, 0.0);
  const size_t h_bytes = result_delta_offset(K, VS) + (size_t)K * B * sizeof(double);
  if (S->h_pinned.reserve(h_bytes))
    return (int)hipErrorOutOfMemory;
  std::memset(S->h_pinned.p, 0, h_bytes);
  const int32_t *base = S->d_int.as<int32_t>();
  SolvePlan &P = S->plan;
  P.K = K; P.B = B; P.Bs = Bs; P.Bp = Bp; P.nblk = nblk; P.nlinks = (int)links.size();
  P.row_first = base + o_rf; P.row_off = base + o_ro;
  P.blk_row = base + o_br; P.blk_col = base + o_bc; P.blk_src = base + o_bs; P.perm = base + o_pm; P.pos = base + o_ps;
  P.to_block = base + o_tb; P.to_solver = base + o_ts;
  S->d_order = base + o_ord;
  S->h_fill.assign((size_t)nblk, 0);
  for (int b = 0; b < nblk; ++b)
    S->h_fill[b] = (blk_src[b] < 0 && blk_row[b] != blk_col[b]) ? 1 : 0;
  S->host_plan = std::move(bp);
  *out = S.release();
  return SAGE_OK;
}

void solver_destroy(DeviceSolver *S) { delete S; }

int solver_set_holds(DeviceSolver *S, const std::vector<uint8_t> &hold, hipStream_t stream)
{
  if ((int)hold.size() != S->K)
    return SAGE_E_INVALID;
  const std::vector<int32_t> masks(hold.begin(), hold.end());
  if (S->d_hold.reserve(masks.size() * sizeof(int32_t)))
    return (int)hipErrorOutOfMemory;
  if (hipMemcpyAsync(S->d_hold.p, masks.data(), masks.size() * sizeof(int32_t), hipMemcpyHostToDevice, stream) != hipSuccess ||
      hipStreamSynchronize(stream) != hipSuccess)
    return (int)hipErrorUnknown;
  S->plan.hold = S->d_hold.as<int32_t>();
  return SAGE_OK;
}

int solver_run(DeviceSolver *S, hipStream_t stream, const double *packed_dev, const float *vars0, float *vars1,
               int CS, double damp, const SolvePriors &pri)
{
  static const bool dbgt = sage::env_flag("SAGE_DEBUG_TIMING");
  hipError_t eh;
  SolveLease lease;
  BlockEnvelope env = envelope_of(S->host_plan, S->Bp);
  if (env.n1 > 0)
    env.no_lookahead = block_chol_arm(block_plan_has_arrow_rows(env), block_plan_long_arrow_chains(env));
  S->epoch += 1;
  if (S->epoch == 0)
    S->epoch = 1;
  hipLaunchKernelGGL(solve_scatter_kernel, dim3(std::min(kScatterWorkgroups, S->nblk)), dim3(256), 0, stream, S->plan,
                     packed_dev, vars0, S->VS, CS, pri, damp, S->h_blocks(), S->h_y, S->d_order,
                     S->h_flags, S->epoch);
  if ((eh = hipGetLastError()) != hipSuccess)
    return (int)eh;
  volatile unsigned *go = &S->result()->go;
  S->go_epoch = (S->go_epoch + 1) & 0x7fffffffu;
  if (S->go_epoch == 0)
    S->go_epoch = 1;
  hipLaunchKernelGGL(solve_retract_kernel, dim3(1), dim3(1024), 0, stream, S->h_y, S->K, S->B, S->Bp, CS, S->VS,
                     S->plan.pos, S->plan.hold, S->plan.to_solver, vars0, vars1, S->host_vars(), S->host_delta(),
                     S->result(), S->go_epoch);
  if ((eh = hipGetLastError()) != hipSuccess)
    return (int)eh;
  struct GoGuard
  {
    volatile unsigned *go;
    unsigned word;
    ~GoGuard()
    {
      std::atomic_thread_fence(std::memory_order_release);
      *go = word;
    }
  } guard{go, S->go_epoch | 0x80000000u};
  const auto t1 = std::chrono::steady_clock::now();
  env.ready = S->h_flags; env.epoch = S->epoch;
  env.fill = S->h_fill.data();
  const int bad = block_chol_solve_tr(env, S->h_blocks(), S->h_X.data(), S->h_y);
  const auto t2 = std::chrono::steady_clock::now();
  if (dbgt)
    fprintf(stderr, "[sage hybrid solve] wait for the system + host cholesky %.3f ms\n",
            std::chrono::duration<double, std::milli>(t2 - t1).count());
  if (bad == -2)
    return SAGE_E_STATE;
  if (bad)
    return SAGE_E_NOT_PSD;
  guard.word = S->go_epoch;
  return SAGE_OK;
}

const float *solver_host_vars(const DeviceSolver *S) { return S->host_vars(); }
const double *solver_host_delta(const DeviceSolver *S) { return S->host_delta(); }
double solver_host_step_norm2(const DeviceSolver *S) { return S->result()->step_norm2; }
int solver_host_status(const DeviceSolver *S) { return S->result()->status; }

SolverLayout solver_layout(const DeviceSolver *S)
{
  return SolverLayout{S->plan.pos, S->plan.to_solver, S->plan.hold, S->Bp, (size_t)S->K * S->Bp};
}

int solver_retract_from(DeviceSolver *S, hipStream_t stream, const double *x_dev, const float *vars0, float *vars1, int CS)
{
  S->go_epoch = (S->go_epoch + 1) & 0x7fffffffu;
  if (S->go_epoch == 0)
    S->go_epoch = 1;
  std::atomic_thread_fence(std::memory_order_release);
  *const_cast<volatile unsigned *>(&S->result()->go) = S->go_epoch;
  hipLaunchKernelGGL(solve_retract_kernel, dim3(1), dim3(1024), 0, stream, x_dev, S->K, S->B, S->Bp, CS, S->VS, S->plan.pos,
                     S->plan.hold, S->plan.to_solver, vars0, vars1, S->host_vars(), S->host_delta(), S->result(), S->go_epoch);
  return (int)hipGetLastError();
}

}
```

sage_slam_amd/csrc/window_build.hip:

```cpp
#include "runtime_internal.h"
#include "window_plan.h"

static std::atomic<int> g_live_windows{0};

extern "C" int sage_window_create(const SageWindowConfig *cfg, void *hip_stream, SageWindow **out)
{
  if (!cfg || !out || !cfg->mask_dev)
    return SAGE_E_INVALID;
  if (!supported(cfg->CS, cfg->FS) || cfg->pyr.levels < 1 || cfg->pyr.levels > SAGE_MAX_LEVELS)
    return SAGE_E_UNSUPPORTED;
  int ndev = 0;
  SAGE_HIP(hipGetDeviceCount(&ndev));
  if (ndev < 1)
    return (int)hipErrorNoDevice;
  SageWindow *w = new SageWindow();
  w->cfg = *cfg;
  w->stream = reinterpret_cast<hipStream_t>(hip_stream);
  w->B = 7 + cfg->CS;
  w->VS = ((13 + cfg->CS + 3) / 4) * 4;
  *out = w;
  g_live_windows.fetch_add(1, std::memory_order_acq_rel);
  return SAGE_OK;
}

extern "C" void sage_window_destroy(SageWindow *w)
{
  if (!w)
    return;
  struct LastOut
  {
    ~LastOut()
    {
      if (g_live_windows.fetch_sub(1, std::memory_order_acq_rel) == 1)
        sage::host_threads_shutdown();
    }
  } last_out;
  std::free(w->dist.rccl_hook);
  sage_shard_plan_destroy(w->dist.shard);
  solver_destroy(w->solver);
  delete w;
}

extern "C" int sage_window_add_keyframe(SageWindow *w, const SageKeyframeView *v, const float *pose12,
                                        const float *code, float scale)
{
  if (!w || !v || !pose12 || !code || w->finalized)
    return SAGE_E_INVALID;
  if (!v->feat_pyr || !v->grad_pyr || !v->bias || !v->basis || !v->loc1d || !v->homo || v->N < 0)
    return SAGE_E_INVALID;
  w->views.push_back(*v);
  for (int s = 0; s < 2; ++s)
  {
    w->hv.pose[s].insert(w->hv.pose[s].end(), pose12, pose12 + 12);
    w->hv.code[s].insert(w->hv.code[s].end(), code, code + w->cfg.CS);
    w->hv.scale[s].push_back(scale);
  }
  w->hv.pose_init.insert(w->hv.pose_init.end(), pose12, pose12 + 12);
  w->hv.code_added.insert(w->hv.code_added.end(), code, code + w->cfg.CS);
  w->hv.scale_init.push_back(scale);
  return w->K++;
}

static int add_link(SageWindow *w, int a, int b, char dense)
{
  if (a == b || a < 0 || b < 0 || a >= w->K || b >= w->K)
    return SAGE_E_INVALID;
  w->links.emplace_back(std::min(a, b), std::max(a, b));
  w->link_geo_loss.push_back(0.f);
  w->link_dense.push_back(dense);
  return (int)w->links.size() - 1;
}

extern "C" int sage_window_add_link(SageWindow *w, int a, int b) { return !w || w->finalized ? SAGE_E_INVALID : add_link(w, a, b, 1); }
extern "C" int sage_window_add_keypoint_link(SageWindow *w, int a, int b)
{
  return !w ? SAGE_E_INVALID : (w->finalized ? SAGE_E_STATE : add_link(w, a, b, 0));
}

extern "C" int sage_window_hold(SageWindow *w, int kf, int what)
{
  if (!w)
    return SAGE_E_INVALID;
  if (w->finalized)
    return SAGE_E_STATE;
  if (kf < 0 || kf >= w->K || what < 0 || what > (SAGE_HOLD_POSE | SAGE_HOLD_CODE | SAGE_HOLD_SCALE))
    return SAGE_E_INVALID;
  w->hold.resize(w->K, 0);
  w->hold[kf] = (uint8_t)what;
  return SAGE_OK;
}

extern "C" int sage_window_set_link_geo_loss(SageWindow *w, int link, float loss_param)
{
  if (!w || w->finalized || link < 0 || link >= (int)w->links.size() || !(loss_param >= 0.f))
    return w && w->finalized ? SAGE_E_STATE : SAGE_E_INVALID;
  w->link_geo_loss[link] = loss_param;
  return SAGE_OK;
}

static int photo_flush_for_runs(int tpb)
{
  if (const char *e = getenv("SAGE_PHOTO_FLUSH"))
    return std::max(0, atoi(e));
  return plan::record_cadence(tpb);
}

static int upload_work_list(DenseSide &sd, const WorkList &wl, hipStream_t s)
{
  int rc;
  sd.n_work = (int)wl.work.size();
  sd.tpb = wl.tiles_per_block;
  if ((rc = upload(sd.work, wl.work, s)) || (rc = upload(sd.first, wl.edge_first, s)) || (rc = upload(sd.tiles, wl.edge_tiles, s)))
    return rc;
  return SAGE_OK;
}

static void window_invalidate_plan_results(SageWindow *w)
{
  w->have_lin = false;
  w->spec_err_valid = false;
  w->dpt_set = -1;
}

static int window_plan_photo_runs(SageWindow *w, int tpb, int flush)
{
  WorkList wp;
  wp.build(w->Nedge, tpb, nullptr, flush);
  int rc;
  w->photo_rec.flush = wp.flush;
  w->photo_rec.n = wp.n_records;
  DenseSide &ph = w->dense[kPhoto];
  if ((rc = upload_work_list(ph, wp, w->stream)) || (rc = upload(w->photo_rec.first, wp.rec_first, w->stream)) ||
      (rc = upload(w->photo_rec.count, wp.rec_count, w->stream)))
    return rc;
  SAGE_HIP(hipStreamSynchronize(w->stream));
  return ph.part.reserve(std::max<size_t>(1, std::max(ph.n_work, w->photo_rec.n)) * photo_partial_floats(w->cfg.CS) * sizeof(float));
}

static std::vector<int> edge_tiles(const std::vector<int> &Nedge)
{
  std::vector<int> tiles;
  for (int n : Nedge)
    tiles.push_back((n + kTile - 1) / kTile);
  return tiles;
}

static int image_pixels(const SageWindow *w) { return (int)w->cfg.pyr.cam[0].h * (int)w->cfg.pyr.cam[0].w; }

static int finalize_variables(SageWindow *w)
{
  const int K = w->K, HW = image_pixels(w);
  int rc;
  for (int s = 0; s < 2; ++s)
  {
    if ((rc = w->vars[s].reserve((size_t)K * w->VS * sizeof(float))))
      return rc;
    if ((rc = window_upload_vars(w, s)))
      return rc;
  }
  if ((rc = w->dpt.reserve((size_t)K * HW * sizeof(float))) || (rc = w->dgrad.reserve((size_t)K * 2 * HW * sizeof(float))))
    return rc;
  return SAGE_OK;
}

static int finalize_ownership(SageWindow *w, FinalizeState &fs)
{
  const int K = w->K, HW = image_pixels(w);
  int rc;
  const bool by_link = sage::env_flag("SAGE_SHARD_BY_LINK") || fs.domain_solve;
  plan::Ownership own = plan::owned_edges((int)w->links.size(), w->rank, w->world, by_link);
  w->owned_edges = std::move(own.edges);
  w->local_links = std::move(own.links);
  w->local_edges = plan::dense_edges(w->owned_edges, w->link_dense);
  fs.needed.assign(K, 0);
  for (int ge : w->local_edges)
    fs.needed[w->links[ge / 2].first] = fs.needed[w->links[ge / 2].second] = 1;
  w->n_depth = 0;
  for (int k = 0; k < K; ++k)
    w->n_depth += fs.needed[k];
  for (int s = 0; s < 2; ++s)
  {
    std::vector<DepthItem> items;
    for (int k = 0; k < K; ++k)
    {
      if (!fs.needed[k])
        continue;
      const float *vp = w->vars[s].as<float>() + (size_t)k * w->VS;
      items.push_back(DepthItem{w->views[k].bias, w->views[k].basis, vp + 13, vp + 12,
                                w->dpt.as<float>() + (size_t)k * HW, w->dgrad.as<float>() + (size_t)k * 2 * HW});
    }
    if ((rc = upload(w->depth_items[s], items, w->stream)))
      return rc;
    SAGE_HIP(hipStreamSynchronize(w->stream));
  }
  return SAGE_OK;
}

static int finalize_pyramids(SageWindow *w)
{
  const SageWindowConfig &c = w->cfg;
  const int FS = c.FS, K = w->K;
  int rc;
  const size_t plane_f = (size_t)FS * c.pyr.P;
  if ((rc = w->pk.reserve((size_t)K * 3 * plane_f * sizeof(float))))
    return rc;
  float lvl_scale[SAGE_MAX_LEVELS] = {};
  for (int l = 0; l < c.pyr.levels; ++l)
  {
    if (!(c.photo_weights[l] >= 0.f))
      return SAGE_E_INVALID;
    lvl_scale[l] = std::sqrt(c.photo_weights[l]);
  }
  for (int k = 0; k < K; ++k)
  {
    float *base = w->pk.as<float>() + (size_t)k * 3 * plane_f;
    SAGE_HIP(launch_repack_groups(w->stream, base, w->views[k].feat_pyr, FS, c.pyr.P, 0, &c.pyr, lvl_scale));
    SAGE_HIP(launch_repack_groups(w->stream, base + plane_f, w->views[k].grad_pyr, FS, c.pyr.P, 1, &c.pyr, lvl_scale));
    SAGE_HIP(launch_repack_groups(w->stream, base + 2 * plane_f, w->views[k].grad_pyr + plane_f, FS, c.pyr.P, 2, &c.pyr, lvl_scale));
  }
// ... 197 lines not shown
        (w->local_edges[e] % 2 == 0 ? fs.le[l].e_ab : fs.le[l].e_ba) = e;
    }
    if ((rc = upload(w->dense[kPhoto].tab[s], pt, w->stream)) || (rc = upload(w->dense[kGeo].tab[s], gt, w->stream)))
      return rc;
    SAGE_HIP(hipStreamSynchronize(w->stream));
  }
  return SAGE_OK;
}

static int finalize_work_lists(SageWindow *w, const FinalizeState &fs)
{
  const std::vector<int> tiles = edge_tiles(fs.Nedge);
  int rc;
  int tpb_g = plan::geo_run(plan::total_tiles(tiles));
  if (const char *e = getenv("SAGE_GEO_TPB"))
    tpb_g = std::max(1, atoi(e));
  WorkList wl;
  wl.build(fs.Nedge, tpb_g);
  if ((rc = upload_work_list(w->dense[kGeo], wl, w->stream)))
    return rc;
  SAGE_HIP(hipStreamSynchronize(w->stream));
  int tpb = plan::photo_run(tiles, w->cfg.FS);
  if (const char *e = getenv("SAGE_PHOTO_TPB"))
    tpb = std::max(1, atoi(e));
  w->Nedge = fs.Nedge;
  w->tpb_heur = tpb;
  if ((rc = window_plan_photo_runs(w, tpb, photo_flush_for_runs(tpb))))
    return rc;
  SAGE_HIP(hipStreamSynchronize(w->stream));
  return SAGE_OK;
}

static int finalize_results(SageWindow *w, const FinalizeState &fs)
{
  const int CS = w->cfg.CS, K = w->K;
  int rc;
  const size_t ne = std::max(1, w->n_edges);
  DenseSide &ph = w->dense[kPhoto], &ge = w->dense[kGeo];
  if ((rc = ph.reserve_results(ne, dense_dim(kPhoto, CS), std::max(ph.n_work, w->photo_rec.n), photo_partial_floats(CS))) ||
      (rc = ge.reserve_results(ne, dense_dim(kGeo, CS), ge.n_work, geo_partial_floats(CS))))
    return rc;
  std::vector<int32_t> adj_start(K + 1, 0);
  std::vector<AdjEntry> adj;
  for (int k = 0; k < K; ++k)
  {
    adj_start[k] = (int32_t)adj.size();
    adj.insert(adj.end(), fs.adjv[k].begin(), fs.adjv[k].end());
  }
  adj_start[K] = (int32_t)adj.size();
  if ((rc = upload(w->adj_start, adj_start, w->stream)) || (rc = upload(w->adj, adj, w->stream)) ||
      (rc = upload(w->link_edges, fs.le, w->stream)))
    return rc;
  SAGE_HIP(hipStreamSynchronize(w->stream));
  if ((rc = w->packed.reserve(sage_window_packed_count(w) * sizeof(double))) || (rc = w->errbuf.reserve(4 * sizeof(double))))
    return rc;
  {
    std::vector<int32_t> ids;
    for (int k = 0; k < K; ++k)
      if (!fs.adjv[k].empty())
        ids.push_back(k);
    for (size_t l = 0; l < fs.le.size(); ++l)
      if (fs.le[l].e_ab >= 0 || fs.le[l].e_ba >= 0 || fs.link_terms[l])
        ids.push_back(K + (int32_t)l);
    ids.push_back(K + (int32_t)w->links.size());
    w->dist.n_asm_blocks = (int)ids.size();
    if ((rc = upload(w->dist.asm_blocks, ids, w->stream)))
      return rc;
    SAGE_HIP(hipStreamSynchronize(w->stream));
  }
  SAGE_HIP(hipMemsetAsync(w->packed.p, 0, sage_window_packed_count(w) * sizeof(double), w->stream));
  SAGE_HIP(hipMemsetAsync(w->errbuf.p, 0, 4 * sizeof(double), w->stream));
  if (!w->mirror.h)
  {
    if ((rc = w->mirror.mem.reserve(TotalsMirror::kDoubles * sizeof(double))))
      return rc;
    w->mirror.h = w->mirror.mem.as<double>();
    std::memset(w->mirror.h, 0, TotalsMirror::kDoubles * sizeof(double));
  }
  w->host_packed.assign(sage_window_packed_count(w), 0.0);
  w->delta.assign((size_t)K * w->B, 0.0);
  return SAGE_OK;
}

static int finalize_solver(SageWindow *w, const FinalizeState &fs)
{
  int rc = solver_create(&w->solver, w->K, w->rows, w->VS, w->links, w->stream);
  if (rc != SAGE_OK && rc != SAGE_E_UNSUPPORTED)
    return rc;
  if (w->solver && window_has_holds(w) && (rc = solver_set_holds(w->solver, w->hold, w->stream)))
    return rc;
  if (!fs.domain_solve)
    return SAGE_OK;
  const std::vector<int32_t> lk = window_link_pairs(w);
  if ((rc = sage_shard_plan_create(w->K, (int)w->links.size(), lk.data(), w->B, w->rank, w->world, &w->dist.shard)))
    return rc;
  const size_t ns = sage_shard_sep_count(w->dist.shard);
  w->dist.h_sep.assign(ns, 0.0);
  if ((rc = w->dist.sepbuf.reserve(ns * sizeof(double))))
    return rc;
  w->host_packed.resize(sage_window_packed_count(w));
  return SAGE_OK;
}

extern "C" int sage_window_finalize(SageWindow *w)
{
  if (!w || w->finalized || w->K < 1)
    return SAGE_E_INVALID;
  FinalizeState fs;
  const char *schur = getenv("SAGE_SHARD_SCHUR");
  fs.domain_solve = plan::uses_domain_solve(w->world, w->K, schur ? atoi(schur) != 0 : -1);
  w->hold.resize(w->K, 0);
  if (fs.domain_solve && (window_has_holds(w) || !w->terms.gt_added.empty()))
    return SAGE_E_UNSUPPORTED;
  w->rows = plan::solver_rows(w->hold.data(), w->K, w->cfg.CS);
  int rc;
  if ((rc = finalize_variables(w)) || (rc = finalize_ownership(w, fs)) || (rc = finalize_pyramids(w)) ||
      (rc = finalize_samples(w)) || (rc = finalize_source_features(w, fs)) || (rc = finalize_edge_tables(w, fs)) ||
      (rc = finalize_terms(w, fs)))
    return rc;
  w->residuals_per_lin = fs.residuals;
  w->bytes_per_lin = fs.bytes;
  if ((rc = finalize_work_lists(w, fs)) || (rc = finalize_results(w, fs)) || (rc = finalize_solver(w, fs)))
    return rc;
  w->finalized = true;
  if (const char *e = getenv("SAGE_AUTOTUNE"))
    if (atoi(e) != 0)
      return sage_window_tune_runs(w, nullptr, nullptr, nullptr, nullptr);
  return SAGE_OK;
}

extern "C" int sage_window_set_runs(SageWindow *w, int tpb)
{
  if (!w || !w->finalized)
    return SAGE_E_STATE;
  if (tpb < 1 || tpb > 64)
    return SAGE_E_INVALID;
  const int rc = window_plan_photo_runs(w, tpb, photo_flush_for_runs(tpb));
  window_invalidate_plan_results(w);
  return rc;
}

extern "C" int sage_window_tune_runs(SageWindow *w, int *tpb_out, int *tpb_rule_out, float *ms_rule_out, float *ms_best_out)
{
  if (!w || !w->finalized)
    return SAGE_E_STATE;
  const int rule = w->tpb_heur;
  if (tpb_out)
    *tpb_out = w->dense[kPhoto].tpb;
  if (tpb_rule_out)
    *tpb_rule_out = rule;
  if (ms_rule_out)
    *ms_rule_out = 0.f;
  if (ms_best_out)
    *ms_best_out = 0.f;
  if (getenv("SAGE_PHOTO_TPB") || w->world > 1 || w->dist.allreduce || w->n_edges == 0 || !(w->cfg.use_photo))
    return SAGE_OK;
  const std::vector<int> cand = plan::tune_candidates(rule, plan::typical_edge(edge_tiles(w->Nedge)));
  const bool prof_was = w->prof.profiling;
  const int level_was = w->prof.prof_level;
  int rc = sage_window_set_profiling(w, 1);
  double best_ms = 0.0, rule_ms = 0.0;
  int best = rule;
  auto measure = [&](int t, double &ms) -> int {
    int r = window_plan_photo_runs(w, t, photo_flush_for_runs(t));
    for (int rep = 0; rep < 4 && !r; ++rep)
    {
      if ((r = sage_window_linearize(w)) || (r = sage_window_error(w, 1)))
        break;
      double lin = 0.0, err = 0.0;
      int nl = 0, ne = 0;
      if ((r = sage_window_get_kernel_time(w, 0, &lin, &nl)) || (r = sage_window_get_kernel_time(w, 2, &err, &ne)))
        break;
// ... 47 lines not shown
```

sage_slam_amd/csrc/window_eval.hip:

```cpp
#include "runtime_internal.h"
#include "finalize_bodies.h"

namespace sage
{

__device__ __forceinline__ int edge_col(int type, int role, int bi, int CS)
{
  if (bi < 6)
    return role * 6 + bi;
  if (type == 2)
    return bi == 6 + CS ? 12 + role : -1;
  if (type == 0)
  {
    if (role == 1)
      return -1;
    return bi < 6 + CS ? 12 + (bi - 6) : 12 + CS;
  }
  if (bi < 6 + CS)
    return 12 + role * CS + (bi - 6);
  return 12 + 2 * CS + role;
}

__device__ __forceinline__ double add_term_errors(double acc, const TermResults &r, bool photo, int lane)
{
  const float *sk = r.stats + (photo ? 0 : 2 * (size_t)r.n_photo_stats());
  const int nk = photo ? r.n_photo_stats() : r.n_geo_stats();
  for (int t = lane; t < nk; t += 64)
    acc += (double)sk[2 * t];
  return acc;
}

template <bool KP>
__global__ __launch_bounds__(1024) void assemble_kernel(const AssembleParams p)
{
  const int B = 7 + p.CS, BB = B * B;
  const int Dp = TermResults::dim(0, p.CS), Dg = TermResults::dim(1, p.CS);
  const int split = p.split > 1 ? p.split : 1;
  const int part = (int)blockIdx.x % split, bslot = (int)blockIdx.x / split;
  const int blk = p.blocks ? p.blocks[bslot] : bslot;
  const int tstride = (int)blockDim.x * split, tfirst = part * (int)blockDim.x + (int)threadIdx.x;
  double *diag = p.packed;
  double *lnk = diag + (size_t)p.K * BB;
  double *g = lnk + (size_t)p.nlinks * BB;
  double *tail = g + (size_t)p.K * B;
  if (blk < p.K)
  {
    const int k = blk;
    const int a0 = p.adj_start[k], a1 = p.adj_start[k + 1];
    constexpr int S = 2;
    for (int base = 0; base < BB + B; base += S * tstride)
    {
    double acc[S] = {0.0, 0.0};
    int bi[S], bj[S];
    bool isg[S], valid[S];
#pragma unroll
    for (int s = 0; s < S; ++s)
    {
      const int idx = base + tfirst + s * tstride;
      valid[s] = idx < BB + B;
      isg[s] = idx >= BB;
      bi[s] = isg[s] ? idx - BB : idx / B;
      bj[s] = isg[s] ? 0 : idx % B;
    }
#pragma unroll 4
    for (int a = a0; a < a1; ++a)
    {
      const AdjEntry ae = p.adj[a];
      const int lt = KP ? adj_group(ae.type) : ae.type;
      const bool kp = KP && ae.type >= 2;
      const int D = TermResults::dim(lt, p.CS);
      const float *A = kp ? p.terms.AtA(lt) : (lt == 0 ? p.AtA_p : p.AtA_g);
      const float *b = kp ? p.terms.Atb(lt) : (lt == 0 ? p.Atb_p : p.Atb_g);
#pragma unroll
      for (int s = 0; s < S; ++s)
      {
        if (!valid[s])
          continue;
        const int ci = edge_col(lt, ae.role, bi[s], p.CS);
        const int cj = isg[s] ? 0 : edge_col(lt, ae.role, bj[s], p.CS);
        if (ci < 0 || cj < 0)
          continue;
        const double *Wd = kp ? nullptr : (lt == 0 ? p.wide_p : p.wide_g);
        if (Wd)
          acc[s] += Wd[(size_t)ae.edge * (D * D + D) + (isg[s] ? (size_t)D * D + ci : (size_t)ci * D + cj)];
// ... 4 lines not shown
#pragma unroll
    for (int s = 0; s < S; ++s)
    {
      const int idx = base + tfirst + s * tstride;
      if (!valid[s])
        continue;
      if (isg[s])
        g[(size_t)k * B + bi[s]] = acc[s];
      else
        diag[(size_t)k * BB + idx] = acc[s];
    }
    }
  }
  else if (blk < p.K + p.nlinks)
  {
    const int l = blk - p.K;
    const LinkEdges le = p.links[l];
    for (int idx = tfirst; idx < BB; idx += tstride)
    {
      const int bi = idx / B, bj = idx % B;
      double acc = 0.0;
      {
        for (int type = 0; type < 2; ++type)
        {
          if ((type == 0 && !p.AtA_p) || (type == 1 && !p.AtA_g))
            continue;
          const int D = type == 0 ? Dp : Dg;
          const float *A = type == 0 ? p.AtA_p : p.AtA_g;
          const double *Wd = type == 0 ? p.wide_p : p.wide_g;
          const size_t ws = (size_t)D * D + D;
          int ci = edge_col(type, 0, bi, p.CS), cj = edge_col(type, 1, bj, p.CS);
          if (le.e_ab >= 0 && ci >= 0 && cj >= 0)
            acc += Wd ? Wd[(size_t)le.e_ab * ws + (size_t)ci * D + cj] : (double)A[(size_t)le.e_ab * D * D + (size_t)ci * D + cj];
          ci = edge_col(type, 1, bi, p.CS);
          cj = edge_col(type, 0, bj, p.CS);
          if (le.e_ba >= 0 && ci >= 0 && cj >= 0)
            acc += Wd ? Wd[(size_t)le.e_ba * ws + (size_t)ci * D + cj] : (double)A[(size_t)le.e_ba * D * D + (size_t)ci * D + cj];
        }
      }
      if (KP && p.link_terms_start)
        for (int a = p.link_terms_start[l]; a < p.link_terms_start[l + 1]; ++a)
        {
          const AdjEntry ae = p.link_terms[a];
          const int lt = adj_group(ae.type), D = TermResults::dim(lt, p.CS);
          const float *A = p.terms.AtA(lt);
          const int ci = edge_col(lt, ae.role, bi, p.CS), cj = edge_col(lt, 1 - ae.role, bj, p.CS);
          if (ci >= 0 && cj >= 0)
            acc += (double)A[(size_t)ae.edge * D * D + (size_t)ci * D + cj];
        }
      lnk[(size_t)l * BB + idx] = acc;
    }
  }
  else
  {
    if (part != 0)
      return;
    const int wave = threadIdx.x >> 6, lane = threadIdx.x & 63;
    const bool photo = (wave & 1) == 0;
    const int which = wave >> 1;
    const float *st = photo ? p.stats_p : p.stats_g;
    const int n = photo ? p.n_edges_p : p.n_edges_g;
    double acc = 0.0;
    if (st && wave < 4)
      for (int e = lane; e < n; e += 64)
        acc += (double)st[2 * e + which];
    if (KP && p.terms.stats && wave < 2)
      acc = add_term_errors(acc, p.terms, photo, lane);
    for (int off = 32; off > 0; off >>= 1)
      acc += __shfl_down(acc, off);
    if (lane == 0 && wave < 4)
    {
      tail[which * 2 + (photo ? 0 : 1)] = acc;
      if (p.tail_mirror)
        p.tail_mirror[which * 2 + (photo ? 0 : 1)] = acc;
    }
  }
}

struct WindowFinalizeParams
{
  PhotoFinalizeParams ph;
  GeoFinalizeParams ge;
  int n_p, n_g;
};

template <int CS>
__global__ __launch_bounds__(kFinalizeBlock) void window_finalize_kernel(const WindowFinalizeParams prm)
{
  constexpr int LDS = photo_finalize_lds_doubles(CS) > geo_finalize_lds_doubles(CS) ? photo_finalize_lds_doubles(CS)
                                                                                    : geo_finalize_lds_doubles(CS);
  __shared__ double s[LDS];
  const int bid = (int)blockIdx.x;
  if (bid < prm.n_g)
    geo_finalize_body<CS>(prm.ge, bid, s);
  else
    photo_finalize_body<CS>(prm.ph, bid - prm.n_g, s);
}

template <bool KP>
__global__ __launch_bounds__(1024) void error_totals_kernel(const ErrorTotalsSide ph, const ErrorTotalsSide ge, double *out,
                                                            double *mirror, double epoch, const TermResults terms)
{
  for (int idx = threadIdx.x; idx < ph.n_edges + ge.n_edges; idx += blockDim.x)
  {
    const bool photo = idx < ph.n_edges;
    const ErrorTotalsSide &sd = photo ? ph : ge;
    const int e = photo ? idx : idx - ph.n_edges;
    const int first = sd.edge_first[e], nt = sd.edge_tiles[e];
    float se = 0.f, sn = 0.f;
    for (int t0 = 0; t0 < nt; t0 += 8)
    {
      float ve[8], vn[8];
#pragma unroll
      for (int u = 0; u < 8; ++u)
      {
        const int t = t0 + u < nt ? t0 + u : nt - 1;
        ve[u] = sd.partials[(size_t)(first + t) * sd.stride + sd.err_off];
        vn[u] = sd.partials[(size_t)(first + t) * sd.stride + sd.cnt_off];
      }
#pragma unroll
      for (int u = 0; u < 8; ++u)
        if (t0 + u < nt)
        {
          se += ve[u];
          sn += vn[u];
        }
    }
    sd.stats[2 * e + 0] = sn > 0.f ? sd.scale * se / sn : sd.fallback;
    sd.stats[2 * e + 1] = sn;
  }
  __threadfence_block();
  __syncthreads();
  const int wave = threadIdx.x >> 6, lane = threadIdx.x & 63;
  if (wave >= 4)
    return;
  const bool photo = (wave & 1) == 0;
  const int which = wave >> 1;
  const ErrorTotalsSide &sd = photo ? ph : ge;
  double acc = 0.0;
  for (int e0 = lane; e0 < sd.n_edges; e0 += 64 * 8)
  {
    float v[8];
#pragma unroll
    for (int u = 0; u < 8; ++u)
    {
      const int e = e0 + 64 * u;
      v[u] = sd.stats[2 * (e < sd.n_edges ? e : lane) + which];
    }
#pragma unroll
    for (int u = 0; u < 8; ++u)
      if (e0 + 64 * u < sd.n_edges)
        acc += (double)v[u];
  }
  if (KP && terms.stats && which == 0)
    acc = add_term_errors(acc, terms, photo, lane);
  for (int off = 32; off > 0; off >>= 1)
    acc += __shfl_down(acc, off);
  if (lane == 0)
  {
    out[which * 2 + (photo ? 0 : 1)] = acc;
    if (mirror)
    {
      mirror[which * 2 + (photo ? 0 : 1)] = acc;
      __threadfence_system();
      *reinterpret_cast<volatile double *>(mirror + 4 + which * 2 + (photo ? 0 : 1)) = epoch;
    }
  }
}

}

static LaunchCommon window_lc(SageWindow *w, int type, bool photo_linearize = false)
{
  const DenseSide &sd = w->dense[type];
  LaunchCommon lc{};
  lc.work = sd.work.as<WorkItem>();
  lc.edge_first = sd.first.as<int32_t>();
  lc.edge_tiles = sd.tiles.as<int32_t>();
  lc.n_work = sd.n_work;
  lc.n_edges = w->n_edges;
  lc.partials = sd.part.as<float>();
  lc.tiles_per_block = sd.tpb;
  lc.packed = type == kPhoto;
  if (photo_linearize && w->photo_rec.flush > 0)
  {
    lc.edge_first = w->photo_rec.first.as<int32_t>();
    lc.edge_tiles = w->photo_rec.count.as<int32_t>();
    lc.flush = w->photo_rec.flush;
  }
  return lc;
}

template <class E, class P>
static void finalize_side(P &fp, const DenseSide &sd, int set, const LaunchCommon &lc)
{
  const EdgeOut out = sd.out();
  fp.table = sd.tab[set].as<E>();
  fp.edge_first = lc.edge_first; fp.edge_tiles = lc.edge_tiles; fp.partials = lc.partials;
  fp.AtA = out.AtA; fp.Atb = out.Atb; fp.stats = out.stats; fp.wide = out.wide;
}

static float photo_weight_sum(const SageWindowConfig &c)
{
  float wsum = 0.f;
  for (int l = 0; l < c.pyr.levels; ++l)
    wsum += c.photo_weights[l];
  return wsum;
}

static AssembleParams window_assemble_params(SageWindow *w)
{
  const SageWindowConfig &c = w->cfg;
  AssembleParams ap{};
  const bool has = w->n_edges > 0;
  const EdgeOut op = w->dense[kPhoto].out(), og = w->dense[kGeo].out();
  ap.AtA_p = (has && c.use_photo) ? op.AtA : nullptr;
  ap.Atb_p = op.Atb;
  ap.stats_p = (has && c.use_photo) ? op.stats : nullptr;
  ap.wide_p = (has && c.use_photo) ? op.wide : nullptr;
  ap.AtA_g = (has && c.use_geo) ? og.AtA : nullptr;
  ap.Atb_g = og.Atb;
  ap.stats_g = (has && c.use_geo) ? og.stats : nullptr;
  ap.wide_g = (has && c.use_geo) ? og.wide : nullptr;
  ap.adj_start = w->adj_start.as<int32_t>();
  ap.adj = w->adj.as<AdjEntry>();
  ap.links = w->link_edges.as<LinkEdges>();
  ap.packed = w->packed.as<double>();
  ap.tail_mirror = w->kernels_mirror_totals() ? w->mirror.h + TotalsMirror::kTail : nullptr;
  ap.K = w->K;
  ap.nlinks = (int)w->links.size();
  ap.CS = c.CS;
  ap.n_edges_p = w->n_edges;
  ap.n_edges_g = w->n_edges;
  ap.split = 1;
  ap.blocks = nullptr;
  ap.terms = w->terms.results(true);
  ap.link_terms_start = w->terms.link_start.as<int32_t>();
  ap.link_terms = w->terms.link.as<AdjEntry>();
  return ap;
}

int window_linearize_set(SageWindow *w, int set, double *dst, bool local_blocks, bool merge)
{
  if (!w || !w->finalized)
    return SAGE_E_STATE;
  const SageWindowConfig &c = w->cfg;
  const int H = (int)c.pyr.cam[0].h, W = (int)c.pyr.cam[0].w;
  const bool dense = w->n_edges > 0;
  LaunchCommon lcg{}, lcp{};
  merge = merge && w->merge_ok;
  if (dense)
  {
    const bool have_depth = w->dpt_set == set;
    SAGE_HIP(launch_depth_batch(w->stream, c.CS, w->depth_items[set].as<DepthItem>(), w->n_depth, H, W, !have_depth,
                                !(have_depth && w->dgrad_valid)));
    w->dpt_set = set;
    w->dgrad_valid = true;
    ++w->dense_serial;
    lcg = window_lc(w, kGeo);
    lcp = window_lc(w, kPhoto, true);
    lcg.stage = 1;
    lcp.stage = 1;
    lcg.merge_geo_weight = lcp.merge_geo_weight = merge ? c.geo_weight : 0.f;
    if (c.use_geo)
    {
      prof_attach(w, 1, lcg);
      SAGE_HIP(launch_geo_linearize(w->stream, c.CS, nullptr, w->dense[kGeo].tab[set].as<GeoEdge>(), lcg, c.pyr.cam[0], c.eps,
                                    c.geo_loss_param, c.geo_weight, w->dense[kGeo].out()));
    }
    if (c.use_photo)
    {
      prof_attach(w, 0, lcp);
      SAGE_HIP(launch_photo_linearize(w->stream, c.CS, c.FS, nullptr, w->dense[kPhoto].tab[set].as<PhotoEdge>(), lcp, c.pyr,
                                      c.photo_weights, c.eps, w->dense[kPhoto].out()));
    }
  }
  if (const int rct = window_launch_terms(w, set, true))
    return rct;
  if (dense)
  {
    WindowFinalizeParams fp{};
    fp.n_p = c.use_photo ? w->n_edges : 0;
    fp.n_g = c.use_geo ? w->n_edges : 0;
    finalize_side<PhotoEdge>(fp.ph, w->dense[kPhoto], set, lcp);
    fp.ph.wsum = photo_weight_sum(c);
    finalize_side<GeoEdge>(fp.ge, w->dense[kGeo], set, lcg);
    fp.ge.weight = c.geo_weight;
    if (merge)
    {
      fp.ge.photo_partials = lcp.partials;
      fp.ge.photo_rec_first = lcp.edge_first;
      fp.ge.photo_rec_count = lcp.edge_tiles;
    }
    if (c.CS == 32)
      hipLaunchKernelGGL((window_finalize_kernel<32>), dim3(fp.n_p + fp.n_g), dim3(kFinalizeBlock), 0, w->stream, fp);
    else
      hipLaunchKernelGGL((window_finalize_kernel<16>), dim3(fp.n_p + fp.n_g), dim3(kFinalizeBlock), 0, w->stream, fp);
    SAGE_HIP(hipGetLastError());
  }
  AssembleParams ap = window_assemble_params(w);
  if (dst)
    ap.packed = dst;
  ap.split = 4;
  int nblocks = w->K + ap.nlinks + 1;
  if (local_blocks && w->dist.n_asm_blocks > 0)
  {
    ap.blocks = w->dist.asm_blocks.as<int32_t>();
    nblocks = w->dist.n_asm_blocks;
  }
  if (ap.terms.stats)
    hipLaunchKernelGGL(assemble_kernel<true>, dim3(nblocks * ap.split), dim3(512), 0, w->stream, ap);
  else
    hipLaunchKernelGGL(assemble_kernel<false>, dim3(nblocks * ap.split), dim3(512), 0, w->stream, ap);
  SAGE_HIP(hipGetLastError());
  window_phase_mark(w, 1);
  if (ap.packed == w->packed.as<double>())
  {
    w->have_lin = true;
    w->lin_epoch = set == 0 ? w->vars_epoch : 0;
    w->spec_err_valid = false;
    w->dist.packed_reduced = false;
    w->dogleg.solved0 = w->dogleg.products = false;
  }
  return SAGE_OK;
}

extern "C" int sage_window_linearize(SageWindow *w)
{
  if (w)
    window_phase_mark(w, 0);
  return window_linearize_set(w, 0);
}

struct PartialRecord
{
  int stride, err_slot, cnt_slot;
};
constexpr PartialRecord kOwnRecord{2, 0, 1};
constexpr PartialRecord kFusedPhoto{4, 0, 1}, kFusedGeo{4, 2, 3};

static ErrorTotalsSide error_totals_side(const LaunchCommon &lc, float *stats, float fallback, float scale, int n_edges,
                                         PartialRecord rec)
{
  ErrorTotalsSide sd{};
  sd.edge_first = lc.edge_first; sd.edge_tiles = lc.edge_tiles; sd.partials = lc.partials;
  sd.stats = stats;
  sd.fallback = fallback; sd.scale = scale;
  sd.n_edges = n_edges;
  sd.stride = rec.stride; sd.err_off = rec.err_slot; sd.cnt_off = rec.cnt_slot;
  return sd;
}

int window_error_pass(SageWindow *w, int which, bool speculate_gradients)
{
  if (!w || !w->finalized || which < 0 || which > 1)
    return SAGE_E_STATE;
  const SageWindowConfig &c = w->cfg;
  const int H = (int)c.pyr.cam[0].h, W = (int)c.pyr.cam[0].w;
  const bool has = w->n_edges > 0;
  if (has && w->dpt_set != which)
  {
    SAGE_HIP(launch_depth_batch(w->stream, c.CS, w->depth_items[which].as<DepthItem>(), w->n_depth, H, W, true, false));
    w->dpt_set = which;
    w->dgrad_valid = false;
  }
  ErrorTotalsSide ph{}, ge{};
  const bool fused = has && c.use_photo && c.use_geo;
  if (has && c.use_photo)
  {
    LaunchCommon lc = window_lc(w, kPhoto);
    prof_attach(w, 2, lc);
    lc.stage = 1;
    lc.fused_geo_loss_param = fused ? c.geo_loss_param : 0.f;
    SAGE_HIP(launch_photo_error(w->stream, c.CS, c.FS, nullptr, w->dense[kPhoto].tab[which].as<PhotoEdge>(), lc, c.pyr,
                                c.photo_weights, c.eps, w->dense[kPhoto].stats.as<float>()));
    ph = error_totals_side(lc, w->dense[kPhoto].stats.as<float>(), 10.0f * photo_weight_sum(c), 1.0f, w->n_edges,
                           fused ? kFusedPhoto : kOwnRecord);
    if (fused)
      ge = error_totals_side(lc, w->dense[kGeo].stats.as<float>(), 10.0f * c.geo_weight, c.geo_weight, w->n_edges, kFusedGeo);
  }
  if (has && c.use_geo && !fused)
  {
    LaunchCommon lc = window_lc(w, kGeo);
    prof_attach(w, 3, lc);
    lc.stage = 1;
    SAGE_HIP(launch_geo_error(w->stream, c.CS, nullptr, w->dense[kGeo].tab[which].as<GeoEdge>(), lc, c.pyr.cam[0], c.eps,
                              c.geo_loss_param, c.geo_weight, w->dense[kGeo].stats.as<float>()));
    ge = error_totals_side(lc, w->dense[kGeo].stats.as<float>(), 10.0f * c.geo_weight, c.geo_weight, w->n_edges, kOwnRecord);
  }
  if (const int rct = window_launch_terms(w, which, false))
    return rct;
  const TermResults kpt = w->terms.results(false);
  w->mirror.err_epoch += 1;
  double *const mirror = w->kernels_mirror_totals() ? w->mirror.h + TotalsMirror::kError : nullptr;
  if (kpt.stats)
    hipLaunchKernelGGL(error_totals_kernel<true>, dim3(1), dim3(1024), 0, w->stream, ph, ge, w->errbuf.as<double>(), mirror,
                       (double)w->mirror.err_epoch, kpt);
  else
    hipLaunchKernelGGL(error_totals_kernel<false>, dim3(1), dim3(1024), 0, w->stream, ph, ge, w->errbuf.as<double>(), mirror,
                       (double)w->mirror.err_epoch, kpt);
  SAGE_HIP(hipGetLastError());
  window_phase_mark(w, 4);
  if (speculate_gradients && has && c.use_geo && w->dpt_set == which && !w->dgrad_valid)
  {
    SAGE_HIP(launch_depth_batch(w->stream, c.CS, w->depth_items[which].as<DepthItem>(), w->n_depth, H, W, false, true));
// ... 7 lines not shown
```

sage_slam_amd/csrc/window_lm.hip:

```cpp
#include "runtime_internal.h"

enum class LmSeq { classic, schur, at_candidate };

static LmSeq lm_sequence_for(const SageWindow *w, const SageLmConfig *cfg)
{
  const bool sharded = w->dist.allreduce != nullptr;
  if (sharded && w->dist.shard)
    return LmSeq::schur;
  const bool at_candidate = cfg->linearize_at_candidate > 0 || (cfg->linearize_at_candidate == 0 && sharded);
  return at_candidate && !w->links.empty() ? LmSeq::at_candidate : LmSeq::classic;
}

struct LmEval
{
  double cur_tot[4];
  bool have_cur_tot;
};

static int window_form_system(SageWindow *w, int set, double *dst, int it)
{
  int rc;
  if (!w->dist.allreduce)
    return (rc = window_linearize_set(w, set, dst, false, true)) ? rc : window_mirror_totals(w, false, dst);
  if ((rc = window_linearize_set(w, set, w->dist.packed_loc.as<double>(), true, true)) ||
// ... 30 lines not shown
    if ((rc = window_form_system(w, 0, w->packed.as<double>(), w->dist.emu_cur)))
      return rc;
    w->have_lin = true;
    w->lin_epoch = w->vars_epoch;
    w->dist.packed_reduced = true;
    w->spec_err_valid = false;
    mirrored_now = true;
  }
  if (!w->spec_err_valid)
  {
    if (!mirrored_now && (rc = window_mirror_totals(w, false)))
      return rc;
    if (!window_wait_reduced_totals(w))
      SAGE_HIP(hipStreamSynchronize(w->stream));
    w->spec_error = mirrored_error(w, TotalsMirror::kTail, 0);
    w->spec_err_valid = true;
  }
  st->error = w->spec_error;
  return SAGE_OK;
}

static int evaluate_schur(SageWindow *w, SageLmState *st, bool first)
{
  int rc;
  double lin_error = 0;
  if ((rc = window_schur_solve(w, st->damp, &lin_error)) && rc != SAGE_E_NOT_PSD)
    return rc;
  window_phase_mark(w, 3);
  if (first)
    st->error = lin_error;
  st->candidate_error = INFINITY;
  if (rc == SAGE_E_NOT_PSD)
    return SAGE_OK;
  if ((rc = sage_window_error(w, 1)))
    return rc;
  window_add_to_double(w, w->errbuf.as<double>(), window_prior_error(w, 1, true));
  if ((rc = window_collective(w, w->errbuf.as<double>(), 4)))
    return rc;
  double t4[4];
  SAGE_HIP(hipMemcpyAsync(t4, w->errbuf.p, sizeof(t4), hipMemcpyDeviceToHost, w->stream));
  SAGE_HIP(hipStreamSynchronize(w->stream));
  st->candidate_error = t4[0] + t4[1];
  return SAGE_OK;
}

static int evaluate_at_candidate(SageWindow *w, SageLmState *st, LmEval &ev)
{
  int rc;
  std::memcpy(ev.cur_tot, w->mirror.h, sizeof(ev.cur_tot));
  ev.have_cur_tot = true;
  bool not_psd;
  if ((rc = window_form_system(w, 1, w->packed_save.as<double>(), w->dist.emu_cur + 1)) ||
      (rc = window_wait_mirror(w, &not_psd)))
    return rc;
  st->candidate_error = not_psd ? INFINITY : mirrored_error(w, TotalsMirror::kTail, 1);
  return SAGE_OK;
}

static int evaluate_classic(SageWindow *w, SageLmState *st, bool first)
{
  int rc;
  const bool sharded = w->dist.allreduce != nullptr;
  if ((rc = window_error_pass(w, 1, !sharded)))
    return rc;
  if (!sharded)
  {
    const bool idle = window_wait_error_totals(w);
    if (first && (rc = window_total_error(w, 1, &st->error, idle)))
      return rc;
    if ((rc = window_total_error(w, 0, &st->candidate_error, idle)) == SAGE_E_NOT_PSD)
      st->candidate_error = INFINITY;
    return rc == SAGE_E_NOT_PSD ? SAGE_OK : rc;
  }
  bool not_psd;
  if ((rc = window_allreduce(w, w->errbuf.as<double>(), 4, w->dist.emu_cur + 1)) || (rc = window_mirror_totals(w, true)) ||
      (rc = window_wait_mirror(w, &not_psd)))
    return rc;
  if (first)
    st->error = mirrored_error(w, TotalsMirror::kTail, 0);
  st->candidate_error = not_psd ? INFINITY : mirrored_error(w, TotalsMirror::kError, 1);
  return SAGE_OK;
}

static int lm_evaluate(LmSeq seq, SageWindow *w, SageLmState *st, bool first, LmEval &ev)
{
  if (seq == LmSeq::schur)
    return evaluate_schur(w, st, first);
  const int rc = sage_window_solve(w, st->damp, nullptr);
  if (rc == SAGE_E_NOT_PSD)
  {
    st->candidate_error = INFINITY;
    return first && seq == LmSeq::classic ? sage_window_total_error(w, 1, &st->error) : SAGE_OK;
  }
  if (rc)
    return rc;
  return seq == LmSeq::at_candidate ? evaluate_at_candidate(w, st, ev) : evaluate_classic(w, st, first);
}

static int lm_accept(LmSeq seq, SageWindow *w, const SageLmState *st)
{
  const int rc = sage_window_accept(w);
  if (rc || seq != LmSeq::at_candidate)
    return rc;
  w->packed.swap(w->packed_save);
  w->lin_epoch = w->vars_epoch;
  w->dist.packed_reduced = true;
  w->spec_error = st->candidate_error;
  return SAGE_OK;
}

static void lm_reject(SageWindow *w, const LmEval &ev)
{
  if (ev.have_cur_tot)
    std::memcpy(w->mirror.h, ev.cur_tot, sizeof(ev.cur_tot));
}

extern "C" int sage_window_lm_step(SageWindow *w, SageLmState *st, const SageLmConfig *cfg)
{
  if (!w || !st || !cfg)
    return SAGE_E_INVALID;
  if (w->world > 1 && !w->dist.allreduce)
    return SAGE_E_STATE;
  const LmSeq seq = lm_sequence_for(w, cfg);
  auto clampd = [&](double d) { return std::min(std::max((double)cfg->min_damp, d), (double)cfg->max_damp); };
  if (st->iters == 0 && st->damp <= 0)
    st->damp = cfg->init_damp;
  window_phase_mark(w, 0);
  int rc = lm_prepare(seq, w, st);
  if (rc)
    return rc;
  st->accepted = 0;
  for (int evals = 1;; ++evals)
  {
    LmEval ev{};
    if ((rc = lm_evaluate(seq, w, st, evals == 1, ev)))
      return rc;
    if (st->candidate_error < st->error)
    {
      st->accepted = 1;
      if ((rc = lm_accept(seq, w, st)))
        return rc;
      st->damp = clampd(st->damp / cfg->damp_dec_factor);
      break;
    }
    lm_reject(w, ev);
    const bool give_up = st->damp >= cfg->max_damp || (cfg->max_inner_evals > 0 && evals >= cfg->max_inner_evals);
    st->damp = clampd(st->damp * cfg->damp_inc_factor);
    if (give_up)
      break;
  }
  st->iters += 1;
  return SAGE_OK;
}

static int window_lm_run(SageWindow *w, SageLmState *st, const SageLmConfig *cfg, int n, double *trace, int *done,
                         double *step_seconds)
{
  if (!w || !st || !cfg || n < 0)
    return SAGE_E_INVALID;
  int i = 0, rc = SAGE_OK;
  auto t_prev = std::chrono::steady_clock::now();
  for (; i < n; ++i)
  {
    if ((rc = sage_window_lm_step(w, st, cfg)))
      break;
    if (trace)
    {
      trace[4 * i + 0] = st->error;
      trace[4 * i + 1] = st->candidate_error;
      trace[4 * i + 2] = (double)st->accepted;
      trace[4 * i + 3] = st->damp;
    }
    if (step_seconds)
    {
      const auto t = std::chrono::steady_clock::now();
      step_seconds[i] = std::chrono::duration<double>(t - t_prev).count();
      t_prev = t;
    }
  }
  if (done)
    *done = i;
  return rc;
}

extern "C" int sage_window_lm_run(SageWindow *w, SageLmState *st, const SageLmConfig *cfg, int n, double *trace, int *done)
{
  return window_lm_run(w, st, cfg, n, trace, done, nullptr);
}

extern "C" int sage_window_lm_run_timed(SageWindow *w, SageLmState *st, const SageLmConfig *cfg, int n, double *trace,
                                        int *done, double *step_seconds)
{
  return window_lm_run(w, st, cfg, n, trace, done, step_seconds);
}
```

sage_slam_amd/csrc/window_profile.hip:

```cpp
#include "runtime_internal.h"

WindowProfiler::~WindowProfiler()
{
  for (auto &pm : phase_pending)
    for (auto &m : pm.ev)
      (void)hipEventDestroy(m.second);
  for (auto &m : phase_cur.ev)
    (void)hipEventDestroy(m.second);
  for (auto &pend : pending)
    for (auto &pr : pend)
    {
      (void)hipEventDestroy(pr.first);
      (void)hipEventDestroy(pr.second);
    }
  for (hipEvent_t e : ev_free)
    (void)hipEventDestroy(e);
}

static bool ev_get(WindowProfiler &pf, hipEvent_t *e)
{
  if (!pf.ev_free.empty())
  {
    *e = pf.ev_free.back();
    pf.ev_free.pop_back();
    return true;
  }
  return hipEventCreate(e) == hipSuccess;
}
static void ev_put(WindowProfiler &pf, hipEvent_t e)
{
  if (e)
    pf.ev_free.push_back(e);
}

void prof_attach(SageWindow *w, int which, LaunchCommon &lc)
{
  WindowProfiler &pf = w->prof;
  if (!pf.profiling || (pf.prof_level == 2 && which != 0))
    return;
  hipEvent_t a, b;
  if (!ev_get(pf, &a))
    return;
  if (!ev_get(pf, &b))
  {
    ev_put(pf, a);
    return;
  }
  lc.ev_start = a;
  lc.ev_stop = b;
  pf.pending[which].emplace_back(a, b);
}

void window_phase_mark(SageWindow *w, int which)
{
  WindowProfiler &pf = w->prof;
  if (!pf.profiling || pf.prof_level == 2)
    return;
  if (which == 0)
  {
    if (pf.phase_cur.ev.size() >= 2)
    {
      if (pf.phase_pending.size() >= 1024)
      {
        for (auto &m : pf.phase_pending.front().ev)
          ev_put(pf, m.second);
        pf.phase_pending.erase(pf.phase_pending.begin());
      }
      pf.phase_pending.push_back(std::move(pf.phase_cur));
    }
    else
      for (auto &m : pf.phase_cur.ev)
        ev_put(pf, m.second);
    pf.phase_cur = WindowProfiler::PhaseMarks{};
  }
  else if (pf.phase_cur.ev.empty())
    return;
  hipEvent_t e;
  if (pf.phase_cur.ev.size() >= 64 || !ev_get(pf, &e))
    return;
  (void)hipEventRecord(e, w->stream);
  pf.phase_cur.ev.emplace_back(which, e);
}

extern "C" int sage_window_get_phase_time(SageWindow *w, double *ms4, int *iterations)
{
  if (!w || !ms4)
    return SAGE_E_INVALID;
  WindowProfiler &pf = w->prof;
  SAGE_HIP(hipStreamSynchronize(w->stream));
  window_phase_mark(w, 0);
  for (auto &m : pf.phase_cur.ev)
    ev_put(pf, m.second);
  pf.phase_cur = WindowProfiler::PhaseMarks{};
  for (auto &pm : pf.phase_pending)
  {
    double d4[4] = {0, 0, 0, 0};
    bool ok = true;
    for (size_t i = 1; i < pm.ev.size() && ok; ++i)
    {
      float d = 0.f;
      ok = hipEventElapsedTime(&d, pm.ev[i - 1].second, pm.ev[i].second) == hipSuccess;
      const int ph = pm.ev[i].first;
      if (ok && ph >= 1 && ph <= 4)
        d4[ph - 1] += d;
    }
    if (ok)
    {
      for (int i = 0; i < 4; ++i)
        pf.phase_ms[i] += d4[i];
      pf.phase_n += 1;
    }
    for (auto &m : pm.ev)
      ev_put(pf, m.second);
  }
  pf.phase_pending.clear();
  for (int i = 0; i < 4; ++i)
  {
    ms4[i] = pf.phase_ms[i];
    pf.phase_ms[i] = 0;
  }
  if (iterations)
    *iterations = pf.phase_n;
  pf.phase_n = 0;
  return SAGE_OK;
}

extern "C" int sage_window_set_profiling(SageWindow *w, int on)
{
  if (!w)
    return SAGE_E_INVALID;
  WindowProfiler &pf = w->prof;
  pf.profiling = on != 0;
  pf.prof_level = on;
  while (pf.profiling && pf.ev_free.size() < 512)
  {
    hipEvent_t e;
    if (hipEventCreate(&e) != hipSuccess)
      break;
    pf.ev_free.push_back(e);
  }
  return SAGE_OK;
}

extern "C" int sage_window_get_kernel_time(SageWindow *w, int which, double *total_ms, int *launches)
{
  if (!w || which < 0 || which > 7)
    return SAGE_E_INVALID;
  WindowProfiler &pf = w->prof;
  SAGE_HIP(hipStreamSynchronize(w->stream));
  for (auto &pr : pf.pending[which])
  {
    float ms = 0.f;
    if (hipEventElapsedTime(&ms, pr.first, pr.second) == hipSuccess)
    {
      pf.prof_ms[which] += ms;
      pf.prof_n[which] += 1;
    }
    ev_put(pf, pr.first);
    ev_put(pf, pr.second);
  }
  pf.pending[which].clear();
  if (total_ms)
    *total_ms = pf.prof_ms[which];
  if (launches)
    *launches = pf.prof_n[which];
  pf.prof_ms[which] = 0;
  pf.prof_n[which] = 0;
  return SAGE_OK;
}
```

sage_slam_amd/csrc/window_state.h:

```cpp
#pragma once

namespace sage_rt
{

enum : int { kPhoto = 0, kGeo = 1 };

static inline size_t dense_dim(int type, int CS) { return type == kPhoto ? 13 + (size_t)CS : 14 + 2 * (size_t)CS; }

struct HostVars
{
  std::vector<float> pose[2], code[2], scale[2];
  std::vector<float> code_init, scale_init, pose_init;
  std::vector<float> code_added;
  void copy_set(int dst, int src) { pose[dst] = pose[src], code[dst] = code[src], scale[dst] = scale[src]; }

  template <class T>
  void pack(int set, int k, int CS, T *rec) const
  {
    for (int i = 0; i < 12; ++i)
      rec[i] = pose[set][(size_t)k * 12 + i];
    rec[12] = scale[set][k];
    for (int i = 0; i < CS; ++i)
      rec[13 + i] = code[set][(size_t)k * CS + i];
  }
// ... 91 lines not shown
};
struct FactorCache
{
  enum : int { kSlots = 2 + plan::kTermGroups, kStatSets = 3 };
  bool lin = false, err = false;
  std::vector<float> pose, code, scale;
  FactorSlot slot[kSlots];
  std::vector<float> stats[kStatSets];
  int psd_mode = -1;
  int psd_launches = 0;
  SagePsdStats psd_worst{};
};

struct PhotoRecordPlan
{
  DevBuf first, count;
  int flush = 0, n = 0;
};

struct TotalsMirror
{
  enum : int { kTail = 0, kError = 4, kErrorTickets = 8, kMirrorTickets = 12, kDoubles = 16 };
  PinnedBuf mem;
  double *h = nullptr;
  uint64_t err_epoch = 0;
  uint64_t mirror_epoch = 0;
  bool wait(int ticket_group, uint64_t epoch) const
  {
    const double *t = h + ticket_group;
    const double want = (double)epoch;
    auto ticket = [t](int i) {
      double v;
      __atomic_load(t + i, &v, __ATOMIC_ACQUIRE);
      return v;
    };
    return spin_until([&] { return ticket(0) == want && ticket(1) == want && ticket(2) == want && ticket(3) == want; });
  }
};

struct DoglegSide
{
  DevBuf tables;
  DevBuf part;
  DevBuf vec;
  DevBuf x;
  PinnedBuf host;
  uint64_t epoch = 0;
  bool ready = false;
  bool solved0 = false;
  bool products = false;
  bool vectors = false;
};

struct WindowDist
{
  SageAllReduceFn allreduce = nullptr;
  int (*allreduce2)(const double *send, double *recv, size_t n, void *user) = nullptr;
  void *allreduce_user = nullptr;
  void *rccl_hook = nullptr;
  SageShardPlan *shard = nullptr;
  DevBuf sepbuf;
  std::vector<double> h_sep;
  const double *emu_rest = nullptr;
  int emu_n = 0, emu_cur = 0;
  DevBuf packed_loc;
  DevBuf asm_blocks;
  int n_asm_blocks = 0;
  bool packed_reduced = false;
};

struct WindowProfiler
{
  struct PhaseMarks
  {
    std::vector<std::pair<int, hipEvent_t>> ev;
  };
  std::vector<PhaseMarks> phase_pending;
  PhaseMarks phase_cur;
  double phase_ms[4] = {0, 0, 0, 0};
  int phase_n = 0;
  bool profiling = false;
  int prof_level = 0;
  std::vector<std::pair<hipEvent_t, hipEvent_t>> pending[8];
  std::vector<hipEvent_t> ev_free;
  double prof_ms[8] = {0, 0, 0, 0, 0, 0, 0, 0};
  int prof_n[8] = {0, 0, 0, 0, 0, 0, 0, 0};
  WindowProfiler() = default;
  WindowProfiler(const WindowProfiler &) = delete;
  WindowProfiler &operator=(const WindowProfiler &) = delete;
  ~WindowProfiler();
};

}
```

Measured before the change: 260,200 Mresiduals/s.

## Split photometric linearize into two parts overlapping with solver scatter and host factorization

Adds a split plan that partitions photo work items, finalize edges and assemble blocks into two parts ordered by the solver's consumption order. The first part is linearized, finalized and assembled, and its prefix of blocks is scattered to the host Cholesky solver before the second part runs. The host block factorization can therefore start consuming early rows while the GPU finishes the rest. It also switches the ready-flag spin to acquire atomics. This adds more kernel launches and partitioning complexity.

```diff
diff --git a/include/sage_ba.h b/include/sage_ba.h
--- a/include/sage_ba.h
+++ b/include/sage_ba.h
@@ -727,6 +727,7 @@
 int sage_window_lm_run(SageWindow *w, SageLmState *st, const SageLmConfig *cfg, int n, double *trace, int *done);
 int sage_window_lm_run_timed(SageWindow *w, SageLmState *st, const SageLmConfig *cfg, int n, double *trace, int *done,
                              double *step_seconds);
+int sage_window_split_info(const SageWindow *w, int *info);
 int sage_window_sync_variables(SageWindow *w);
 
 enum { SAGE_DOGLEG_SEARCH_EACH_ITERATION = 0, SAGE_DOGLEG_SEARCH_REDUCE_ONLY = 1, SAGE_DOGLEG_ONE_STEP_PER_ITERATION = 2 };
diff --git a/sage_slam_amd/build.py b/sage_slam_amd/build.py
--- a/sage_slam_amd/build.py
+++ b/sage_slam_amd/build.py
@@ -12,7 +12,7 @@
 LIB = os.path.join(HERE, "libsage_ba.so")
 SOURCES = ["photo_kernels.hip", "geo_kernels.hip", "track_kernels.hip", "producers.hip", "keypoint_kernels.hip", "graph_kernels.hip", "solve_kernels.hip", "operators.hip", "tracker.hip", "overlap.hip", "depth_scale.hip", "bow.hip", "registration.hip", "match_batch.hip", "voc_build.hip", "window.hip", "window_eval.hip", "window_reduce.hip", "window_solve.hip", "window_lm.hip", "window_profile.hip", "window_build.hip", "window_terms.hip", "window_dist.hip", "window_factors.hip", "psd_project.hip", "window_dogleg.hip",
            "host_math.cpp", "factor_blocks.cpp", "block_solver.cpp", "host_threads.cpp", "shard_solve.cpp", "convex_hull.cpp", "bow_database.cpp", "registration_host.cpp", "voc_build_host.cpp", "depth_scale_host.cpp", "loop_accept_host.cpp", "psd_project_host.cpp", "dogleg_host.cpp"]
-HEADERS = ["sage_device.h", "sage_internal.h", "damped_system.h", "host_math.h", "factor_blocks.h", "block_solver.h", "host_threads.h", "device_buffers.h", "runtime_internal.h", "window_state.h", "finalize_bodies.h", "keypoint_batch.h", "graph_terms.h", "graph_batch.h", "term_results.h", "window_plan.h", "registration_plan.h", "registration_math.h", "depth_scale_plan.h", "loop_accept.h", "voc_build.h", "psd_project.h", "dogleg.h", os.path.join(ROOT, "include", "sage_ba.h")]
+HEADERS = ["sage_device.h", "sage_internal.h", "damped_system.h", "host_math.h", "factor_blocks.h", "block_solver.h", "host_threads.h", "device_buffers.h", "runtime_internal.h", "window_state.h", "finalize_bodies.h", "keypoint_batch.h", "graph_terms.h", "graph_batch.h", "term_results.h", "window_plan.h", "split_plan.h", "solver_call.h", "registration_plan.h", "registration_math.h", "depth_scale_plan.h", "loop_accept.h", "voc_build.h", "psd_project.h", "dogleg.h", os.path.join(ROOT, "include", "sage_ba.h")]
 HIPCC = os.environ.get("HIPCC", "/opt/rocm/bin/hipcc")
 HOSTCXX = os.environ.get("HOSTCXX", "/opt/rocm/lib/llvm/bin/clang++")
 FLAGS = ["--offload-arch=gfx950", "-O3", "-std=c++17", "-fPIC", "-Wall", "-Wno-unused-function",
diff --git a/sage_slam_amd/capi.py b/sage_slam_amd/capi.py
--- a/sage_slam_amd/capi.py
+++ b/sage_slam_amd/capi.py
@@ -193,7 +193,7 @@
     "sage_window_block_size", "sage_window_solver_block_size", "sage_window_packed_count", "sage_window_packed_dev",
     "sage_window_residuals_per_linearize", "sage_window_bytes_per_linearize", "sage_window_linearize",
     "sage_window_error", "sage_window_tune_runs", "sage_window_set_runs", "sage_window_error_dev", "sage_window_solve", "sage_window_total_error",
-    "sage_window_accept", "sage_window_reset", "sage_window_get_keyframe", "sage_window_set_keyframe", "sage_window_get_delta",
+    "sage_window_split_info", "sage_window_accept", "sage_window_reset", "sage_window_get_keyframe", "sage_window_set_keyframe", "sage_window_get_delta",
     "sage_window_get_edge", "sage_window_add_keypoint_term", "sage_window_num_keypoint_terms", "sage_window_get_keypoint_term", "sage_window_add_graph_term", "sage_window_num_graph_terms", "sage_window_get_graph_term", "sage_window_prepass", "sage_window_factor", "sage_window_factor_error", "sage_term_factor_block_count", "sage_term_factor_blocks", "sage_window_keypoint_factor", "sage_window_keypoint_factor_error", "sage_window_graph_factor", "sage_window_graph_factor_error", "sage_window_prepare_factors", "sage_window_prepare_factors_device", "sage_window_prepare_factors_device_launches", "sage_factor_psd", "sage_factor_psd_batch", "sage_factor_psd_batch_launches", "sage_factor_psd_batch_plan", "sage_jacobi_round_pairs", "sage_factor_cut_blocks", "sage_window_set_profiling", "sage_window_get_kernel_time", "sage_window_get_phase_time", "sage_window_lm_step", "sage_window_lm_run", "sage_window_lm_run_timed", "sage_window_sync_variables", "sage_window_set_allreduce", "sage_shard_plan_create", "sage_shard_plan_create_domains", "sage_block_solve_domains", "sage_shard_plan_destroy", "sage_shard_sep_count", "sage_shard_num_separators", "sage_shard_num_interior", "sage_shard_keyframe_owner", "sage_shard_keyframe_is_local", "sage_shard_eliminate", "sage_shard_solve", "sage_rccl_unique_id", "sage_rccl_comm_create", "sage_rccl_comm_destroy", "sage_rccl_comm_info", "sage_window_use_rccl", "sage_window_emulate_peers", "sage_sort_locations", "sage_bind_thread_to_device", "sage_solver_helper_cpus", "sage_solver_placement_moves", "sage_placement_monitor", "sage_shutdown", "sage_host_threads_running",
     "sage_valid_locations", "sage_shuffle_indices", "sage_sample_locations",
     "sage_reprojection_jac_error_calculate", "sage_reprojection_error_calculate",
@@ -1449,6 +1449,11 @@
                                             C.byref(done), sec.ctypes.data_as(C.POINTER(C.c_double))), "sage_window_lm_run_timed")
         return tr[:done.value], sec[:done.value]
 
+    def split_info(self):
+        v = (C.c_int * 5)()
+        _chk(lib().sage_window_split_info(self.h, v), "sage_window_split_info")
+        return dict(rows=v[0], edges=v[1], work_items=v[2], order_prefix=v[3], evaluations=v[4])
+
     def dogleg_step(self, state: SageDoglegState, cfg: SageDoglegConfig):
         _chk(lib().sage_window_dogleg_step(self.h, C.byref(state), C.byref(cfg)), "sage_window_dogleg_step")
         return state
diff --git a/sage_slam_amd/csrc/block_solver.cpp b/sage_slam_amd/csrc/block_solver.cpp
--- a/sage_slam_amd/csrc/block_solver.cpp
+++ b/sage_slam_amd/csrc/block_solver.cpp
@@ -325,12 +325,13 @@
   }
   if (!E.ready)
     return true;
-  const volatile unsigned *f = E.ready + idx;
-  if (!peek || *f != E.epoch)
+  const unsigned *f = const_cast<const unsigned *>(E.ready) + idx;
+  auto ticket = [f] { return __atomic_load_n(f, __ATOMIC_ACQUIRE); };
+  if (!peek || ticket() != E.epoch)
   {
     const double t0 = mono_seconds();
     unsigned spins = 0;
-    while (*f != E.epoch)
+    while (ticket() != E.epoch)
     {
       __builtin_ia32_pause();
       if ((++spins & 0xfff) == 0 && ((abort && abort->load(std::memory_order_acquire)) || mono_seconds() - t0 > 2.0))
@@ -1345,6 +1346,7 @@
   for (int k = 0; k < K; ++k)
     perm[k] = k;
   n1 = n2 = 0;
+  out.n_cover = 0;
   for (auto &l : links)
     if (l.first < 0 || l.second <= l.first || l.second >= K)
       return SAGE_E_INVALID;
@@ -1408,11 +1410,13 @@
       std::sort(cover.begin(), cover.end());
       for (int k : cover)
         perm[q++] = k;
+      out.n_cover = (int)cover.size();
       if (n1 < 1 || n2 < 1)
       {
         for (int k = 0; k < K; ++k)
           perm[k] = k;
         n1 = n2 = 0;
+        out.n_cover = 0;
       }
     }
   }
diff --git a/sage_slam_amd/csrc/block_solver.h b/sage_slam_amd/csrc/block_solver.h
--- a/sage_slam_amd/csrc/block_solver.h
+++ b/sage_slam_amd/csrc/block_solver.h
@@ -73,6 +73,7 @@
   std::vector<int32_t> perm, pos, row_first, row_off, a_first, a_cnt, a_off, blk_row, blk_col, blk_src;
   std::vector<int32_t> col_ptr, col_rows;
   int nblk = 0, n1 = 0, n2 = 0;
+  int n_cover = 0;
   int index(int i, int j) const
   {
     return j < row_first[i] ? a_off[i] + j - a_first[i] : row_off[i] + j - row_first[i];
diff --git a/sage_slam_amd/csrc/runtime_internal.h b/sage_slam_amd/csrc/runtime_internal.h
--- a/sage_slam_amd/csrc/runtime_internal.h
+++ b/sage_slam_amd/csrc/runtime_internal.h
@@ -45,6 +45,7 @@
 #include "depth_scale_plan.h"
 #include "loop_accept.h"
 #include "dogleg.h"
+#include "solver_call.h"
 
 using namespace sage;
 
@@ -249,6 +250,17 @@
   float fallback, scale;
   int n_edges;
   int stride, err_off, cnt_off;
+};
+
+struct SplitSide
+{
+  int rows = 0;
+  int order_prefix = 0;
+  int n_work[2] = {0, 0}, n_edges[2] = {0, 0}, n_blocks[2] = {0, 0};
+  DevBuf work;
+  DevBuf edges;
+  DevBuf blocks;
+  long long evaluations = 0;
 };
 
 }
@@ -306,6 +318,7 @@
   FactorCache fc;
   uint64_t dense_serial = 0;
   DoglegSide dogleg;
+  sage::SplitSide split;
   WindowProfiler prof;
 
   bool kernels_mirror_totals() const { return world == 1 && !dist.allreduce && mirror.h; }
@@ -339,10 +352,13 @@
   std::vector<char> link_terms;
   double residuals = 0, bytes = 0;
 };
+int window_plan_split(SageWindow *w);
 int finalize_terms(SageWindow *w, FinalizeState &fs);
 int window_launch_terms(SageWindow *w, int set, bool jac);
 int window_linearize_set(SageWindow *w, int set, double *dst = nullptr, bool local_blocks = false, bool merge = false);
 int window_error_pass(SageWindow *w, int which, bool speculate_gradients);
+bool window_split_ready(const SageWindow *w);
+int window_linearize_solve_split(SageWindow *w, double damp, int *solve_rc);
 int window_collective(SageWindow *w, double *buf, size_t n);
 int window_allreduce(SageWindow *w, double *buf, size_t n, int iterate);
 int window_allreduce_into(SageWindow *w, const double *send, double *recv, size_t n, int iterate);
@@ -358,5 +374,5 @@
 SolvePriors window_solve_priors(const SageWindow *w);
 int window_sync_candidate(SageWindow *w, bool stream_idle = false);
 int window_schur_solve(SageWindow *w, double damp, double *lin_error);
-void prof_attach(SageWindow *w, int which, LaunchCommon &lc);
+void prof_attach(SageWindow *w, int which, LaunchCommon &lc, bool continuation = false);
 void window_phase_mark(SageWindow *w, int which);
diff --git a/sage_slam_amd/csrc/solve_kernels.hip b/sage_slam_amd/csrc/solve_kernels.hip
--- a/sage_slam_amd/csrc/solve_kernels.hip
+++ b/sage_slam_amd/csrc/solve_kernels.hip
@@ -13,6 +13,8 @@
 #include "sage_device.h"
 #include "sage_internal.h"
 #include "window_plan.h"
+#include "split_plan.h"
+#include "solver_call.h"
 
 namespace sage
 {
@@ -43,8 +45,8 @@
                                                             const float *__restrict__ vars0, int VS, int CS,
                                                             const SolvePriors pri, double damp,
                                                             double *__restrict__ L, double *__restrict__ y,
-                                                            const int32_t *__restrict__ order, unsigned *flags,
-                                                            unsigned epoch)
+                                                            const int32_t *__restrict__ order, int count,
+                                                            unsigned *flags, unsigned epoch)
 {
   const int tid = threadIdx.x;
   const int B = P.B, Bs = P.Bs, Bp = P.Bp, BB = B * B;
@@ -53,7 +55,7 @@
   if (tid < Bs)
     s_row[tid] = P.to_block[tid];
   __syncthreads();
-  for (int it = blockIdx.x; it < P.nblk; it += gridDim.x)
+  for (int it = blockIdx.x; it < count; it += gridDim.x)
   {
     const int b = order[it];
     const int i = P.blk_row[b], j = P.blk_col[b], srcf = P.blk_src[b];
@@ -233,10 +235,9 @@
   const int rcp = plan_blocks(K, links, !sage::env_flag("SAGE_SOLVE_NO_SPLIT"), bp);
   if (rcp != SAGE_OK)
     return rcp;
-  const int n1 = bp.n1, n2 = bp.n2, nblk = bp.nblk;
+  const int nblk = bp.nblk;
   const std::vector<int32_t> &perm = bp.perm, &pos = bp.pos, &row_first = bp.row_first, &row_off = bp.row_off,
-                             &a_cnt = bp.a_cnt, &a_off = bp.a_off, &blk_row = bp.blk_row, &blk_col = bp.blk_col,
-                             &blk_src = bp.blk_src;
+                             &blk_row = bp.blk_row, &blk_col = bp.blk_col, &blk_src = bp.blk_src;
   std::unique_ptr<DeviceSolver> S(new DeviceSolver);
   S->K = K; S->B = B; S->Bs = Bs; S->Bp = Bp; S->nblk = nblk; S->nlinks = (int)links.size(); S->VS = VS;
   std::vector<int32_t> all;
@@ -249,28 +250,7 @@
   };
   const size_t o_rf = put(row_first), o_ro = put(row_off), o_br = put(blk_row), o_bc = put(blk_col),
                o_bs = put(blk_src), o_pm = put(perm), o_ps = put(pos);
-  std::vector<int32_t> order;
-  auto push_row = [&](int i) {
-    for (int q = 0; q < a_cnt[i]; ++q)
-      order.push_back(a_off[i] + q);
-    for (int q = 0; q <= i - row_first[i]; ++q)
-      order.push_back(row_off[i] + q);
-  };
-  if (n1 > 0)
-  {
-    for (int t = 0; t < std::max(n1, n2); ++t)
-    {
-      if (t < n1)
-        push_row(t);
-      if (t < n2)
-        push_row(n1 + t);
-    }
-    for (int i = n1 + n2; i < K; ++i)
-      push_row(i);
-  }
-  else
-    for (int i = 0; i < K; ++i)
-      push_row(i);
+  const std::vector<int32_t> order = plan::consumption_order(bp);
   const size_t o_ord = put(order);
   const size_t o_tb = put(rows.to_block), o_ts = put(rows.to_solver);
   if (S->d_int.reserve(all.size() * sizeof(int32_t)))
@@ -321,43 +301,74 @@
   return SAGE_OK;
 }
 
-int solver_run(DeviceSolver *S, hipStream_t stream, const double *packed_dev, const float *vars0, float *vars1,
-               int CS, double damp, const SolvePriors &pri)
-{
-  static const bool dbgt = sage::env_flag("SAGE_DEBUG_TIMING");
-  hipError_t eh;
+struct SolveCall
+{
   SolveLease lease;
-  BlockEnvelope env = envelope_of(S->host_plan, S->Bp);
-  if (env.n1 > 0)
-    env.no_lookahead = block_chol_arm(block_plan_has_arrow_rows(env), block_plan_long_arrow_chains(env));
+  DeviceSolver *S = nullptr;
+  hipStream_t stream = nullptr;
+  const double *packed_dev = nullptr;
+  const float *vars0 = nullptr;
+  float *vars1 = nullptr;
+  int CS = 0;
+  double damp = 0.0;
+  SolvePriors pri{};
+  BlockEnvelope env;
+  volatile unsigned *go = nullptr;
+  unsigned word = 0;
+  ~SolveCall()
+  {
+    if (go)
+    {
+      std::atomic_thread_fence(std::memory_order_release);
+      *go = word;
+    }
+  }
+};
+void SolveCallEnd::operator()(SolveCall *c) const { delete c; }
+
+int solver_begin(DeviceSolver *S, hipStream_t stream, const double *packed_dev, const float *vars0, float *vars1, int CS,
+                 double damp, const SolvePriors &pri, SolveCallPtr &out)
+{
+  out.reset(new SolveCall);
+  SolveCall &c = *out;
+  c.S = S; c.stream = stream; c.packed_dev = packed_dev; c.vars0 = vars0; c.vars1 = vars1; c.CS = CS; c.damp = damp; c.pri = pri;
+  c.env = envelope_of(S->host_plan, S->Bp);
+  if (c.env.n1 > 0)
+    c.env.no_lookahead = block_chol_arm(block_plan_has_arrow_rows(c.env), block_plan_long_arrow_chains(c.env));
   S->epoch += 1;
   if (S->epoch == 0)
     S->epoch = 1;
-  hipLaunchKernelGGL(solve_scatter_kernel, dim3(std::min(kScatterWorkgroups, S->nblk)), dim3(256), 0, stream, S->plan,
-                     packed_dev, vars0, S->VS, CS, pri, damp, S->h_blocks(), S->h_y, S->d_order,
+  return SAGE_OK;
+}
+
+int solver_enqueue_range(SolveCall *c, int first, int count)
+{
+  DeviceSolver *S = c->S;
+  if (first < 0 || count < 1 || first + count > S->nblk)
+    return SAGE_E_INVALID;
+  hipLaunchKernelGGL(solve_scatter_kernel, dim3(std::min(kScatterWorkgroups, count)), dim3(256), 0, c->stream, S->plan,
+                     c->packed_dev, c->vars0, S->VS, c->CS, c->pri, c->damp, S->h_blocks(), S->h_y, S->d_order + first, count,
                      S->h_flags, S->epoch);
-  if ((eh = hipGetLastError()) != hipSuccess)
-    return (int)eh;
-  volatile unsigned *go = &S->result()->go;
+  return (int)hipGetLastError();
+}
+
+int solver_end(SolveCall *c)
+{
+  static const bool dbgt = sage::env_flag("SAGE_DEBUG_TIMING");
+  DeviceSolver *S = c->S;
+  hipError_t eh;
   S->go_epoch = (S->go_epoch + 1) & 0x7fffffffu;
   if (S->go_epoch == 0)
     S->go_epoch = 1;
-  hipLaunchKernelGGL(solve_retract_kernel, dim3(1), dim3(1024), 0, stream, S->h_y, S->K, S->B, S->Bp, CS, S->VS,
-                     S->plan.pos, S->plan.hold, S->plan.to_solver, vars0, vars1, S->host_vars(), S->host_delta(),
+  hipLaunchKernelGGL(solve_retract_kernel, dim3(1), dim3(1024), 0, c->stream, S->h_y, S->K, S->B, S->Bp, c->CS, S->VS,
+                     S->plan.pos, S->plan.hold, S->plan.to_solver, c->vars0, c->vars1, S->host_vars(), S->host_delta(),
                      S->result(), S->go_epoch);
   if ((eh = hipGetLastError()) != hipSuccess)
     return (int)eh;
-  struct GoGuard
-  {
-    volatile unsigned *go;
-    unsigned word;
-    ~GoGuard()
-    {
-      std::atomic_thread_fence(std::memory_order_release);
-      *go = word;
-    }
-  } guard{go, S->go_epoch | 0x80000000u};
+  c->go = &S->result()->go;
+  c->word = S->go_epoch | 0x80000000u;
   const auto t1 = std::chrono::steady_clock::now();
+  BlockEnvelope &env = c->env;
   env.ready = S->h_flags; env.epoch = S->epoch;
   env.fill = S->h_fill.data();
   const int bad = block_chol_solve_tr(env, S->h_blocks(), S->h_X.data(), S->h_y);
@@ -369,9 +380,22 @@
     return SAGE_E_STATE;
   if (bad)
     return SAGE_E_NOT_PSD;
-  guard.word = S->go_epoch;
+  c->word = S->go_epoch;
   return SAGE_OK;
 }
+
+int solver_run(DeviceSolver *S, hipStream_t stream, const double *packed_dev, const float *vars0, float *vars1,
+               int CS, double damp, const SolvePriors &pri)
+{
+  SolveCallPtr call;
+  int rc;
+  if ((rc = solver_begin(S, stream, packed_dev, vars0, vars1, CS, damp, pri, call)) ||
+      (rc = solver_enqueue_range(call.get(), 0, S->nblk)))
+    return rc;
+  return solver_end(call.get());
+}
+
+const BlockPlan &solver_block_plan(const DeviceSolver *S) { return S->host_plan; }
 
 const float *solver_host_vars(const DeviceSolver *S) { return S->host_vars(); }
 const double *solver_host_delta(const DeviceSolver *S) { return S->host_delta(); }
diff --git a/sage_slam_amd/csrc/solver_call.h b/sage_slam_amd/csrc/solver_call.h
--- /dev/null
+++ b/sage_slam_amd/csrc/solver_call.h
@@ -0,0 +1,23 @@
+#pragma once
+
+#include <memory>
+
+#include "sage_internal.h"
+
+namespace sage
+{
+
+struct SolveCall;
+struct SolveCallEnd
+{
+  void operator()(SolveCall *c) const;
+};
+using SolveCallPtr = std::unique_ptr<SolveCall, SolveCallEnd>;
+int solver_begin(DeviceSolver *S, hipStream_t stream, const double *packed_dev, const float *vars0, float *vars1, int CS,
+                 double damp, const SolvePriors &pri, SolveCallPtr &out);
+int solver_enqueue_range(SolveCall *c, int first, int count);
+int solver_end(SolveCall *c);
+struct BlockPlan;
+const BlockPlan &solver_block_plan(const DeviceSolver *S);
+
+}
diff --git a/sage_slam_amd/csrc/split_plan.h b/sage_slam_amd/csrc/split_plan.h
--- /dev/null
+++ b/sage_slam_amd/csrc/split_plan.h
@@ -0,0 +1,160 @@
+#pragma once
+
+#include <stdint.h>
+
+#include <algorithm>
+#include <utility>
+#include <vector>
+
+#include "block_solver.h"
+
+namespace sage
+{
+namespace plan
+{
+
+constexpr int kSplitFifths = 4;
+inline int default_split_rows(int n1, int n2) { return kSplitFifths * std::min(n1, n2) / 5; }
+
+inline std::vector<int32_t> consumption_order(const BlockPlan &bp)
+{
+  const int K = (int)bp.perm.size(), n1 = bp.n1, n2 = bp.n2;
+  std::vector<int32_t> order;
+  auto push_row = [&](int i) {
+    for (int q = 0; q < bp.a_cnt[i]; ++q)
+      order.push_back(bp.a_off[i] + q);
+    for (int q = 0; q <= i - bp.row_first[i]; ++q)
+      order.push_back(bp.row_off[i] + q);
+  };
+  if (n1 > 0)
+  {
+    for (int t = 0; t < std::max(n1, n2); ++t)
+    {
+      if (t < n1)
+        push_row(t);
+      if (t < n2)
+        push_row(n1 + t);
+    }
+    for (int i = n1 + n2; i < K; ++i)
+      push_row(i);
+  }
+  else
+    for (int i = 0; i < K; ++i)
+      push_row(i);
+  return order;
+}
+
+struct SplitPlan
+{
+  int rows = 0;
+  int order_prefix = 0;
+  std::vector<int32_t> blocks[2];
+  std::vector<int32_t> edges[2];
+  bool split() const { return rows > 0; }
+};
+
+inline SplitPlan split_plan(const BlockPlan &bp, int rows, const std::vector<std::vector<int32_t>> &kf_edges,
+                            const std::vector<std::pair<int32_t, int32_t>> &link_edges, int n_edges)
+{
+  SplitPlan sp;
+  const int K = (int)bp.perm.size(), n1 = bp.n1, n2 = bp.n2, nlinks = (int)link_edges.size();
+  if (n1 <= 0 || n2 <= 0 || rows <= 0 || rows >= n1 || (int)kf_edges.size() != K)
+    return sp;
+  const int r1 = rows, r2 = std::min(rows, n2);
+  auto in_p1 = [&](int i) { return i < r1 || (i >= n1 && i < n1 + r2); };
+  for (int b = 0; b < bp.nblk; ++b)
+    if (in_p1(bp.blk_row[b]) && !in_p1(bp.blk_col[b]))
+      return sp;
+  long long reach = 0;
+  for (int i = n1 + n2; i < K; ++i)
+    reach += bp.a_cnt[i] + (n1 + n2) - std::min((int)bp.row_first[i], n1 + n2);
+  if (bp.n_cover > 0 || reach > 64)
+    return sp;
+  std::vector<char> e1(std::max(n_edges, 0), 0), blk1((size_t)K + nlinks, 0);
+  int prefix = 0;
+  const std::vector<int32_t> order = consumption_order(bp);
+  for (int32_t b : order)
+  {
+    if (!in_p1(bp.blk_row[b]))
+      break;
+    ++prefix;
+  }
+  for (int it = 0; it < (int)order.size(); ++it)
+    if ((it < prefix) != in_p1(bp.blk_row[order[it]]))
+      return sp;
+  auto take = [&](int32_t e) {
+    if (e >= 0 && e < n_edges)
+      e1[e] = 1;
+  };
+  for (int it = 0; it < prefix; ++it)
+  {
+    const int b = order[it], i = bp.blk_row[b], j = bp.blk_col[b], srcf = bp.blk_src[b];
+    if (i == j)
+    {
+      const int kf = bp.perm[i];
+      blk1[kf] = 1;
+      for (int32_t e : kf_edges[kf])
+        take(e);
+    }
+    else if (srcf >= 0)
+    {
+      const int l = srcf & 0x3fffffff;
+      if (l >= nlinks)
+        return sp;
+      blk1[(size_t)K + l] = 1;
+      take(link_edges[l].first);
+      take(link_edges[l].second);
+    }
+  }
+  for (int e = 0; e < n_edges; ++e)
+    sp.edges[e1[e] ? 0 : 1].push_back(e);
+  for (int b = 0; b < K + nlinks; ++b)
+    sp.blocks[blk1[b] ? 0 : 1].push_back(b);
+  sp.blocks[1].push_back(K + nlinks);
+  if (sp.edges[0].empty() || sp.edges[1].empty() || sp.blocks[0].empty() || prefix <= 0 || prefix >= (int)order.size())
+  {
+    sp = SplitPlan();
+    return sp;
+  }
+  sp.rows = rows;
+  sp.order_prefix = prefix;
+  return sp;
+}
+
+inline std::vector<int32_t> split_work_order(const std::vector<int32_t> &item_edge, const std::vector<int32_t> &edges_first,
+                                             int n_edges, int *n_first)
+{
+  const int n = (int)item_edge.size();
+  std::vector<char> first(std::max(n_edges, 0), 0);
+  for (int32_t e : edges_first)
+    if (e >= 0 && e < n_edges)
+      first[e] = 1;
+  std::vector<int32_t> order, second;
+  for (int i = 0; i < n; ++i)
+    (first[item_edge[i]] ? order : second).push_back(i);
+  int nf = (int)order.size();
+  if (nf % 8 != 0)
+  {
+    int q = 0, best = -1;
+    while (q < (int)second.size())
+    {
+      int q1 = q;
+      while (q1 < (int)second.size() && item_edge[second[q1]] == item_edge[second[q]])
+        ++q1;
+      q = q1;
+      if ((nf + q) % 8 == 0 && q < (int)second.size())
+      {
+        best = q;
+        break;
+      }
+    }
+    if (best > 0)
+      nf += best;
+  }
+  order.insert(order.end(), second.begin(), second.end());
+  *n_first = nf;
+  return order;
+}
+
+}
+}
diff --git a/sage_slam_amd/csrc/window_build.hip b/sage_slam_amd/csrc/window_build.hip
--- a/sage_slam_amd/csrc/window_build.hip
+++ b/sage_slam_amd/csrc/window_build.hip
@@ -1,5 +1,6 @@
 #include "runtime_internal.h"
 #include "window_plan.h"
+#include "split_plan.h"
 
 static std::atomic<int> g_live_windows{0};
 
@@ -134,7 +135,9 @@
       (rc = upload(w->photo_rec.count, wp.rec_count, w->stream)))
     return rc;
   SAGE_HIP(hipStreamSynchronize(w->stream));
-  return ph.part.reserve(std::max<size_t>(1, std::max(ph.n_work, w->photo_rec.n)) * photo_partial_floats(w->cfg.CS) * sizeof(float));
+  if ((rc = ph.part.reserve(std::max<size_t>(1, std::max(ph.n_work, w->photo_rec.n)) * photo_partial_floats(w->cfg.CS) * sizeof(float))))
+    return rc;
+  return w->finalized ? window_plan_split(w) : SAGE_OK;
 }
 
 static std::vector<int> edge_tiles(const std::vector<int> &Nedge)
@@ -498,12 +501,87 @@
   return SAGE_OK;
 }
 
+int window_plan_split(SageWindow *w)
+{
+  SplitSide &sp = w->split;
+  sp.rows = 0;
+  const char *sw = getenv("SAGE_LM_SPLIT");
+  if (!sw || atoi(sw) == 0 || !w->solver || w->world != 1 || w->n_edges < 2 || !w->cfg.use_photo || w->photo_rec.flush <= 0 ||
+      !w->terms.gt_added.empty() || !w->terms.kp_added.empty() || window_has_holds(w) || (int)w->local_edges.size() != w->n_edges)
+    return SAGE_OK;
+  const BlockPlan &bp = solver_block_plan(w->solver);
+  const int K = w->K, nl = (int)w->links.size(), ne = w->n_edges;
+  std::vector<std::vector<int32_t>> kf_edges(K);
+  std::vector<std::pair<int32_t, int32_t>> link_edges(nl, {-1, -1});
+  for (int e = 0; e < ne; ++e)
+  {
+    const int ge = w->local_edges[e], l = ge / 2;
+    kf_edges[w->links[l].first].push_back(e);
+    kf_edges[w->links[l].second].push_back(e);
+    (ge % 2 == 0 ? link_edges[l].first : link_edges[l].second) = e;
+  }
+  int rows = plan::default_split_rows(bp.n1, bp.n2);
+  if (const char *e = getenv("SAGE_LM_SPLIT_ROWS"))
+    rows = atoi(e);
+  const plan::SplitPlan P = plan::split_plan(bp, rows, kf_edges, link_edges, ne);
+  if (!P.split())
+    return SAGE_OK;
+  const DenseSide &ph = w->dense[kPhoto];
+  WorkList wl;
+  wl.build(w->Nedge, ph.tpb, nullptr, w->photo_rec.flush);
+  if ((int)wl.work.size() != ph.n_work)
+    return SAGE_OK;
+  std::vector<int32_t> item_edge(wl.work.size());
+  for (size_t i = 0; i < wl.work.size(); ++i)
+    item_edge[i] = wl.work[i].edge;
+  int n_first = 0;
+  const std::vector<int32_t> order = plan::split_work_order(item_edge, P.edges[0], ne, &n_first);
+  if (n_first <= 0 || n_first >= (int)order.size())
+    return SAGE_OK;
+  std::vector<WorkItem> work(order.size());
+  for (size_t i = 0; i < order.size(); ++i)
+    work[i] = wl.work[order[i]];
+  std::vector<int32_t> edges(P.edges[0]), blocks(P.blocks[0]);
+  edges.insert(edges.end(), P.edges[1].begin(), P.edges[1].end());
+  blocks.insert(blocks.end(), P.blocks[1].begin(), P.blocks[1].end());
+  int rc;
+  if ((rc = upload(sp.work, work, w->stream)) || (rc = upload(sp.edges, edges, w->stream)) ||
+      (rc = upload(sp.blocks, blocks, w->stream)))
+    return rc;
+  SAGE_HIP(hipStreamSynchronize(w->stream));
+  sp.n_work[0] = n_first;
+  sp.n_work[1] = (int)order.size() - n_first;
+  for (int h = 0; h < 2; ++h)
+  {
+    sp.n_edges[h] = (int)P.edges[h].size();
+    sp.n_blocks[h] = (int)P.blocks[h].size();
+  }
+  sp.order_prefix = P.order_prefix;
+  sp.rows = P.rows;
+  return SAGE_OK;
+}
+
+extern "C" int sage_window_split_info(const SageWindow *w, int *info)
+{
+  if (!w || !info)
+    return SAGE_E_INVALID;
+  const SplitSide &sp = w->split;
+  info[0] = sp.rows;
+  info[1] = sp.rows ? sp.n_edges[0] : 0;
+  info[2] = sp.rows ? sp.n_work[0] : 0;
+  info[3] = sp.rows ? sp.order_prefix : 0;
+  info[4] = (int)std::min<long long>(sp.evaluations, 0x7fffffff);
+  return SAGE_OK;
+}
+
 static int finalize_solver(SageWindow *w, const FinalizeState &fs)
 {
   int rc = solver_create(&w->solver, w->K, w->rows, w->VS, w->links, w->stream);
   if (rc != SAGE_OK && rc != SAGE_E_UNSUPPORTED)
     return rc;
   if (w->solver && window_has_holds(w) && (rc = solver_set_holds(w->solver, w->hold, w->stream)))
+    return rc;
+  if ((rc = window_plan_split(w)))
     return rc;
   if (!fs.domain_solve)
     return SAGE_OK;
diff --git a/sage_slam_amd/csrc/window_eval.hip b/sage_slam_amd/csrc/window_eval.hip
--- a/sage_slam_amd/csrc/window_eval.hip
+++ b/sage_slam_amd/csrc/window_eval.hip
@@ -1,5 +1,6 @@
 #include "runtime_internal.h"
 #include "finalize_bodies.h"
+#include "block_solver.h"
 
 namespace sage
 {
@@ -170,6 +171,7 @@
   PhotoFinalizeParams ph;
   GeoFinalizeParams ge;
   int n_p, n_g;
+  const int32_t *edges;
 };
 
 template <int CS>
@@ -179,10 +181,12 @@
                                                                                     : geo_finalize_lds_doubles(CS);
   __shared__ double s[LDS];
   const int bid = (int)blockIdx.x;
+  const int slot = bid < prm.n_g ? bid : bid - prm.n_g;
+  const int e = prm.edges ? prm.edges[slot] : slot;
   if (bid < prm.n_g)
-    geo_finalize_body<CS>(prm.ge, bid, s);
+    geo_finalize_body<CS>(prm.ge, e, s);
   else
-    photo_finalize_body<CS>(prm.ph, bid - prm.n_g, s);
+    photo_finalize_body<CS>(prm.ph, e, s);
 }
 
 template <bool KP>
@@ -328,6 +332,51 @@
   return ap;
 }
 
+static int window_launch_finalize(SageWindow *w, int set, const LaunchCommon &lcp, const LaunchCommon &lcg, bool merge,
+                                  const int32_t *edges = nullptr, int n = 0)
+{
+  const SageWindowConfig &c = w->cfg;
+  const int ne = edges ? n : w->n_edges;
+  WindowFinalizeParams fp{};
+  fp.n_p = c.use_photo ? ne : 0;
+  fp.n_g = c.use_geo ? ne : 0;
+  fp.edges = edges;
+  finalize_side<PhotoEdge>(fp.ph, w->dense[kPhoto], set, lcp);
+  fp.ph.wsum = photo_weight_sum(c);
+  finalize_side<GeoEdge>(fp.ge, w->dense[kGeo], set, lcg);
+  fp.ge.weight = c.geo_weight;
+  if (merge)
+  {
+    fp.ge.photo_partials = lcp.partials;
+    fp.ge.photo_rec_first = lcp.edge_first;
+    fp.ge.photo_rec_count = lcp.edge_tiles;
+  }
+  if (c.CS == 32)
+    hipLaunchKernelGGL((window_finalize_kernel<32>), dim3(fp.n_p + fp.n_g), dim3(kFinalizeBlock), 0, w->stream, fp);
+  else
+    hipLaunchKernelGGL((window_finalize_kernel<16>), dim3(fp.n_p + fp.n_g), dim3(kFinalizeBlock), 0, w->stream, fp);
+  return (int)hipGetLastError();
+}
+
+static int window_launch_assemble(SageWindow *w, AssembleParams &ap, int nblocks)
+{
+  ap.split = 4;
+  if (ap.terms.stats)
+    hipLaunchKernelGGL(assemble_kernel<true>, dim3(nblocks * ap.split), dim3(512), 0, w->stream, ap);
+  else
+    hipLaunchKernelGGL(assemble_kernel<false>, dim3(nblocks * ap.split), dim3(512), 0, w->stream, ap);
+  return (int)hipGetLastError();
+}
+
+static void window_book_linearize(SageWindow *w, int set)
+{
+  w->have_lin = true;
+  w->lin_epoch = set == 0 ? w->vars_epoch : 0;
+  w->spec_err_valid = false;
+  w->dist.packed_reduced = false;
+  w->dogleg.solved0 = w->dogleg.products = false;
+}
+
 int window_linearize_set(SageWindow *w, int set, double *dst, bool local_blocks, bool merge)
 {
   if (!w || !w->finalized)
@@ -367,48 +416,105 @@
     return rct;
   if (dense)
   {
-    WindowFinalizeParams fp{};
-    fp.n_p = c.use_photo ? w->n_edges : 0;
-    fp.n_g = c.use_geo ? w->n_edges : 0;
-    finalize_side<PhotoEdge>(fp.ph, w->dense[kPhoto], set, lcp);
-    fp.ph.wsum = photo_weight_sum(c);
-    finalize_side<GeoEdge>(fp.ge, w->dense[kGeo], set, lcg);
-    fp.ge.weight = c.geo_weight;
-    if (merge)
-    {
-      fp.ge.photo_partials = lcp.partials;
-      fp.ge.photo_rec_first = lcp.edge_first;
-      fp.ge.photo_rec_count = lcp.edge_tiles;
-    }
-    if (c.CS == 32)
-      hipLaunchKernelGGL((window_finalize_kernel<32>), dim3(fp.n_p + fp.n_g), dim3(kFinalizeBlock), 0, w->stream, fp);
-    else
-      hipLaunchKernelGGL((window_finalize_kernel<16>), dim3(fp.n_p + fp.n_g), dim3(kFinalizeBlock), 0, w->stream, fp);
-    SAGE_HIP(hipGetLastError());
+    if (const int rcf = window_launch_finalize(w, set, lcp, lcg, merge))
+      return rcf;
   }
   AssembleParams ap = window_assemble_params(w);
   if (dst)
     ap.packed = dst;
-  ap.split = 4;
   int nblocks = w->K + ap.nlinks + 1;
   if (local_blocks && w->dist.n_asm_blocks > 0)
   {
     ap.blocks = w->dist.asm_blocks.as<int32_t>();
     nblocks = w->dist.n_asm_blocks;
   }
-  if (ap.terms.stats)
-    hipLaunchKernelGGL(assemble_kernel<true>, dim3(nblocks * ap.split), dim3(512), 0, w->stream, ap);
-  else
-    hipLaunchKernelGGL(assemble_kernel<false>, dim3(nblocks * ap.split), dim3(512), 0, w->stream, ap);
-  SAGE_HIP(hipGetLastError());
+  if (const int rca = window_launch_assemble(w, ap, nblocks))
+    return rca;
   window_phase_mark(w, 1);
   if (ap.packed == w->packed.as<double>())
-  {
-    w->have_lin = true;
-    w->lin_epoch = set == 0 ? w->vars_epoch : 0;
-    w->spec_err_valid = false;
-    w->dist.packed_reduced = false;
-    w->dogleg.solved0 = w->dogleg.products = false;
+    window_book_linearize(w, set);
+  return SAGE_OK;
+}
+
+bool window_split_ready(const SageWindow *w)
+{
+  return w->finalized && w->split.rows > 0 && w->solver && w->world == 1 && !w->dist.allreduce && w->n_edges > 0;
+}
+
+int window_linearize_solve_split(SageWindow *w, double damp, int *solve_rc)
+{
+  if (!w || !solve_rc || !window_split_ready(w))
+    return SAGE_E_STATE;
+  const SageWindowConfig &c = w->cfg;
+  const int H = (int)c.pyr.cam[0].h, W = (int)c.pyr.cam[0].w, set = 0;
+  const SplitSide &sp = w->split;
+  int rc = window_sync_candidate(w);
+  if (rc && rc != SAGE_E_NOT_PSD)
+    return rc;
+  const bool merge = w->merge_ok;
+  const bool have_depth = w->dpt_set == set;
+  SAGE_HIP(launch_depth_batch(w->stream, c.CS, w->depth_items[set].as<DepthItem>(), w->n_depth, H, W, !have_depth,
+                              !(have_depth && w->dgrad_valid)));
+  w->dpt_set = set;
+  w->dgrad_valid = true;
+  ++w->dense_serial;
+  LaunchCommon lcg = window_lc(w, kGeo), lcp = window_lc(w, kPhoto, true);
+  lcg.stage = 1;
+  lcp.stage = 1;
+  lcg.merge_geo_weight = lcp.merge_geo_weight = merge ? c.geo_weight : 0.f;
+  if (c.use_geo)
+  {
+    prof_attach(w, 1, lcg);
+    SAGE_HIP(launch_geo_linearize(w->stream, c.CS, nullptr, w->dense[kGeo].tab[set].as<GeoEdge>(), lcg, c.pyr.cam[0], c.eps,
+                                  c.geo_loss_param, c.geo_weight, w->dense[kGeo].out()));
+  }
+  if ((rc = window_launch_terms(w, set, true)))
+    return rc;
+  AssembleParams ap = window_assemble_params(w);
+  SolveCallPtr call;
+  const int n_order = solver_block_plan(w->solver).nblk;
+  int first_work = 0, first_edge = 0, first_block = 0, first_order = 0;
+  for (int part = 0; part < 2; ++part)
+  {
+    LaunchCommon lc = lcp;
+    lc.work = sp.work.as<WorkItem>() + first_work;
+    lc.n_work = sp.n_work[part];
+    prof_attach(w, 0, lc, part == 1);
+    SAGE_HIP(launch_photo_linearize(w->stream, c.CS, c.FS, nullptr, w->dense[kPhoto].tab[set].as<PhotoEdge>(), lc, c.pyr,
+                                    c.photo_weights, c.eps, w->dense[kPhoto].out()));
+    if ((rc = window_launch_finalize(w, set, lcp, lcg, merge, sp.edges.as<int32_t>() + first_edge, sp.n_edges[part])))
+      return rc;
+    ap.blocks = sp.blocks.as<int32_t>() + first_block;
+    if ((rc = window_launch_assemble(w, ap, sp.n_blocks[part])))
+      return rc;
+    if (part == 1)
+    {
+      window_phase_mark(w, 1);
+      window_book_linearize(w, set);
+      window_phase_mark(w, 2);
+    }
+    else if ((rc = solver_begin(w->solver, w->stream, w->packed.as<double>(), w->vars[0].as<float>(), w->vars[1].as<float>(), c.CS,
+                                damp, window_solve_priors(w), call)))
+      return rc;
+    const int n_scatter = part == 0 ? sp.order_prefix : n_order - sp.order_prefix;
+    if ((rc = solver_enqueue_range(call.get(), first_order, n_scatter)))
+      return rc;
+    first_work += sp.n_work[part];
+    first_edge += sp.n_edges[part];
+    first_block += sp.n_blocks[part];
+    first_order += n_scatter;
+  }
+  rc = solver_end(call.get());
+  call.reset();
+  w->split.evaluations += 1;
+  if (rc && rc != SAGE_E_NOT_PSD)
+    return rc;
+  *solve_rc = rc;
+  if (rc == SAGE_OK)
+  {
+    w->dogleg.solved0 = damp == 0.0;
+    window_phase_mark(w, 3);
+    w->cand_pending = true;
   }
   return SAGE_OK;
 }
diff --git a/sage_slam_amd/csrc/window_lm.hip b/sage_slam_amd/csrc/window_lm.hip
--- a/sage_slam_amd/csrc/window_lm.hip
+++ b/sage_slam_amd/csrc/window_lm.hip
@@ -136,11 +136,11 @@
   return SAGE_OK;
 }
 
-static int lm_evaluate(LmSeq seq, SageWindow *w, SageLmState *st, bool first, LmEval &ev)
+static int lm_evaluate(LmSeq seq, SageWindow *w, SageLmState *st, bool first, LmEval &ev, const int *solved = nullptr)
 {
   if (seq == LmSeq::schur)
     return evaluate_schur(w, st, first);
-  const int rc = sage_window_solve(w, st->damp, nullptr);
+  const int rc = solved ? *solved : sage_window_solve(w, st->damp, nullptr);
   if (rc == SAGE_E_NOT_PSD)
   {
     st->candidate_error = INFINITY;
@@ -180,14 +180,16 @@
   if (st->iters == 0 && st->damp <= 0)
     st->damp = cfg->init_damp;
   window_phase_mark(w, 0);
-  int rc = lm_prepare(seq, w, st);
+  const bool split = seq == LmSeq::classic && window_split_ready(w);
+  int solved = SAGE_OK;
+  int rc = split ? window_linearize_solve_split(w, st->damp, &solved) : lm_prepare(seq, w, st);
   if (rc)
     return rc;
   st->accepted = 0;
   for (int evals = 1;; ++evals)
   {
     LmEval ev{};
-    if ((rc = lm_evaluate(seq, w, st, evals == 1, ev)))
+    if ((rc = lm_evaluate(seq, w, st, evals == 1, ev, split && evals == 1 ? &solved : nullptr)))
       return rc;
     if (st->candidate_error < st->error)
     {
diff --git a/sage_slam_amd/csrc/window_profile.hip b/sage_slam_amd/csrc/window_profile.hip
--- a/sage_slam_amd/csrc/window_profile.hip
+++ b/sage_slam_amd/csrc/window_profile.hip
@@ -33,7 +33,7 @@
     pf.ev_free.push_back(e);
 }
 
-void prof_attach(SageWindow *w, int which, LaunchCommon &lc)
+void prof_attach(SageWindow *w, int which, LaunchCommon &lc, bool continuation)
 {
   WindowProfiler &pf = w->prof;
   if (!pf.profiling || (pf.prof_level == 2 && which != 0))
@@ -49,6 +49,8 @@
   lc.ev_start = a;
   lc.ev_stop = b;
   pf.pending[which].emplace_back(a, b);
+  if (continuation)
+    pf.continued.push_back(a);
 }
 
 void window_phase_mark(SageWindow *w, int which)
@@ -151,10 +153,14 @@
   for (auto &pr : pf.pending[which])
   {
     float ms = 0.f;
+    const auto cont = std::find(pf.continued.begin(), pf.continued.end(), pr.first);
+    const bool continues = cont != pf.continued.end();
+    if (continues)
+      pf.continued.erase(cont);
     if (hipEventElapsedTime(&ms, pr.first, pr.second) == hipSuccess)
     {
       pf.prof_ms[which] += ms;
-      pf.prof_n[which] += 1;
+      pf.prof_n[which] += continues ? 0 : 1;
     }
     ev_put(pf, pr.first);
     ev_put(pf, pr.second);
diff --git a/sage_slam_amd/csrc/window_state.h b/sage_slam_amd/csrc/window_state.h
--- a/sage_slam_amd/csrc/window_state.h
+++ b/sage_slam_amd/csrc/window_state.h
@@ -197,6 +197,7 @@
   bool profiling = false;
   int prof_level = 0;
   std::vector<std::pair<hipEvent_t, hipEvent_t>> pending[8];
+  std::vector<hipEvent_t> continued;
   std::vector<hipEvent_t> ev_free;
   double prof_ms[8] = {0, 0, 0, 0, 0, 0, 0, 0};
   int prof_n[8] = {0, 0, 0, 0, 0, 0, 0, 0};
```

Result: no change. 261,000 Mresiduals/s (median of 3 runs) (+0.3%).
